# armlabstanford/Touch-GS

Hardware: AMD Instinct MI355X
Metric: train iters/s (whole-job views/s) + render Mpix/s, 1M Gaussians @ 1080p (higher is better)
Workload: dtype f32; 1 GPU; configs[2]: 1M Gaussians, 1080p, full Touch-GS train loop (RGB L1/SSIM + tactile depth/uncertainty loss), one view per rank per iter; gaussians=1000000, width=1920, height=1080, sh_degree=3, views=8, tiles=8160, longest_tile_list_any_view=792, max_list_hint=1022, parallelism=dp1, layout=morton (model.spatial_sort(): same scene, rows permuted), depth_loss_type=DEPTH_UNCERTAINTY_WEIGHTED_LOSS

## Files before the change

include/tgs.h:

```cpp
#ifndef TGS_H
#define TGS_H
#include <stddef.h>
#include <stdint.h>

#ifdef __cplusplus
extern "C" {
#endif

#define TGS_VERSION 320
#define TGS_BLOCK 16
#define TGS_SPLAT_FLOATS 12
#define TGS_PARTIAL_FLOATS 12
#define TGS_GROUP 256

typedef enum TgsStatus {
  TGS_OK = 0,
  TGS_E_ARG = -1,
  TGS_E_HIP = -2,
  TGS_E_CAPACITY = -3
} TgsStatus;

typedef struct TgsCamera {
  float viewmat[16];
  float fx, fy, cx, cy;
  int32_t W, H;
  float near_plane;
  float pix_center;
  float bg[3];
  float glob_scale;
  int32_t long_run;
} TgsCamera;

typedef struct TgsLossSpec {
  const float* gt_rgb;
  const float* gt_depth;
  const float* uncertainty;
  float l1_weight;
  float depth_weight;
  float uncertainty_weight;
  float eps;
} TgsLossSpec;

typedef struct TgsAdamSpec {
  float lr_means, lr_scales, lr_quats, lr_opac, lr_sh_dc, lr_sh_rest;
  float beta1, beta2, eps;
  float bias_corr1, bias_corr2;
  const float* device_bias_corr;
} TgsAdamSpec;

int tgs_version(void);
const char* tgs_last_error(void);

int tgs_calib_fma_stream(int n_iter, float* sink, int64_t* n_wave_instr , void* stream);

int tgs_num_groups(int N);
int tgs_num_tiles(int W, int H);
int tgs_num_bands(int W, int H);
int tgs_band_tiles(int W, int H, int band, int* tile0, int* tile1);
int tgs_tile_order_len(int W, int H);
int tgs_tile_counter_len(int W, int H);
int64_t tgs_tile_start_len(int W, int H);
size_t tgs_sort_scratch_bytes(int64_t capacity);

int tgs_project_fwd(const TgsCamera* cam , int N, const float* means,
                    const float* log_scales, const float* quats, const float* opac_logit,
                    const float* sh, int sh_stride, int sh_deg, const float* colors_in,
                    float* splats, int32_t* radii, void* stream);

int tgs_sh_fwd(int N, int sh_deg, int sh_stride, const float* dirs, const float* coeffs,
               float* colors, void* stream);
int tgs_sh_bwd(int N, int sh_deg, int sh_stride, const float* dirs, const float* v_colors,
               float* v_coeffs, void* stream);

int tgs_bin_sort(const TgsCamera* cam , int N, float* splats, int32_t* group_base,
                 int32_t* tile_start, int64_t tile_start_len, int32_t* tile_cursor, int32_t* sorted_gid,
                 int32_t* tile_order, int64_t capacity, void* scratch, int32_t* status,
                 int32_t* sticky_overflow, int32_t max_list_hint, void* stream);

int tgs_project_bin_sort(const TgsCamera* cam , int N, const float* means,
                         const float* log_scales, const float* quats, const float* opac_logit,
                         const float* sh, int sh_stride, int sh_deg, float* splats, int32_t* radii,
                         int32_t* group_base, int32_t* tile_start, int64_t tile_start_len, int32_t* tile_cursor,
                         int32_t* sorted_gid, int32_t* tile_order, int64_t capacity, void* scratch,
                         int32_t* status, int32_t* sticky_overflow, int32_t max_list_hint, void* stream);

int tgs_project_bin_sort_colors(const TgsCamera* cam , int N, const float* means,
                                const float* log_scales, const float* quats, const float* opac_logit,
                                const float* sh, int sh_stride, int sh_deg, float* splats,
                                int32_t* radii, int32_t* group_base, int32_t* tile_start, int64_t tile_start_len,
                                int32_t* tile_cursor, int32_t* sorted_gid, int32_t* tile_order,
                                int64_t capacity, void* scratch, int32_t* status,
                                int32_t* sticky_overflow, int32_t max_list_hint, const float* colors_in,
                                const int32_t* color_tag, int32_t tag_expect, void* stream);

typedef struct TgsRasterOpts {
  int32_t k6_blocks;
  int32_t k6_split;
  int32_t k7_front_to_back;
  int32_t k7_quad;
  int32_t k7_quad_min_walk;
  int32_t k7_blocks;
  int32_t k6_split_floor;
  int32_t k6_split_heads;
} TgsRasterOpts;

int tgs_rasterize_fwd(const TgsCamera* cam , const float* splats,
                      const int32_t* sorted_gid, int32_t* tile_start, int64_t tile_start_len,
                      const int32_t* tile_order, float* out_rgb, float* out_depth, float* final_T,
                      int32_t* final_idx , int32_t* stop_pos ,
                      uint64_t* slot_ok , const TgsRasterOpts* opts ,
                      void* stream);
size_t tgs_slot_ok_len(int W, int H, int64_t capacity);

int tgs_rasterize_depth_stats(const TgsCamera* cam , const float* splats, const int32_t* sorted_gid,
                              const int32_t* tile_start, int64_t tile_start_len, const int32_t* tile_order ,
                              const float* out_depth, const float* final_T, const int32_t* stop_pos ,
                              float* depth_var, float* median_depth, int32_t* median_gid ,
                              const TgsRasterOpts* opts , void* stream);

int tgs_set_raster_variant(int k6_blocks_on, int k7_front_to_back);

int tgs_set_k7_quad(int factor, int min_walk);

int tgs_set_k7_scan(int min_walk, int heads);

int tgs_set_long_run(int tiles);

int tgs_set_k6_split(int factor);
int tgs_set_k6_split_shape(int floor, int heads);

int tgs_rasterize_bwd(const TgsCamera* cam , const float* splats,
                      const int32_t* group_base, const int32_t* sorted_gid,
                      int32_t* tile_start, int64_t tile_start_len, const int32_t* tile_order ,
                      const float* out_rgb, const float* out_depth, const float* final_T,
                      const int32_t* stop_pos, const float* v_rgb, const float* v_depth, const float* v_alpha,
                      const TgsLossSpec* loss , float* partials, float* tile_loss,
                      const uint64_t* slot_ok , const TgsRasterOpts* opts ,
                      void* stream);

int tgs_rasterize_bwd_band(const TgsCamera* cam , const float* splats,
                      const int32_t* group_base, const int32_t* sorted_gid,
                      int32_t* tile_start, int64_t tile_start_len, const int32_t* tile_order ,
                      const float* out_rgb, const float* out_depth, const float* final_T,
                      const int32_t* stop_pos, const float* v_rgb, const float* v_depth, const float* v_alpha,
                      const TgsLossSpec* loss , float* partials, float* tile_loss,
                      int band, const uint64_t* slot_ok ,
                      const TgsRasterOpts* opts , void* stream);

int tgs_reduce_partials(int N, const float* splats, const int32_t* group_base,
                        const TgsCamera* cam , const float* partials, float* v_splats,
                        void* stream);

int tgs_project_bwd(const TgsCamera* cam , int N, const float* means,
                    const float* log_scales, const float* quats, const float* opac_logit,
                    const float* sh, int sh_stride, int sh_deg, const float* splats,
                    const int32_t* group_base, const float* partials, const float* v_splats,
                    float* v_means, float* v_log_scales, float* v_quats, float* v_opac_logit,
                    float* v_sh, float* v_xy,
                    const int32_t* skip_if_overflow , void* stream);

int tgs_project_bwd_adam(const TgsCamera* cam , int N, int sh_stride, int sh_deg,
                         float* params, float* exp_avg, float* exp_avg_sq,
                         const TgsAdamSpec* spec , const float* splats,
                         const int32_t* group_base, const float* partials, float* v_xy,
                         const int32_t* skip_if_overflow ,
                         void* stream);

int tgs_project_bwd_adam_next(const TgsCamera* cam , int N, int sh_stride, int sh_deg,
                              float* params, float* exp_avg, float* exp_avg_sq,
                              const TgsAdamSpec* spec , const float* splats,
                              const int32_t* group_base, const float* partials, float* v_xy,
                              const int32_t* skip_if_overflow ,
                              const TgsCamera* next_cam , float* colors_next,
                              int32_t* color_tag, int32_t tag_value, void* stream);

int tgs_project_bwd_adam_next_front(const TgsCamera* cam , int N, int sh_stride, int sh_deg,
                                    float* params, float* exp_avg, float* exp_avg_sq,
                                    const TgsAdamSpec* spec , const float* splats,
                                    const int32_t* group_base, const float* partials, float* v_xy,
                                    const int32_t* skip_if_overflow ,
                                    const TgsCamera* next_cam , float* colors_next,
                                    int32_t* tag_word, int32_t tag_value, float* splats_next,
                                    int32_t* radii_next, int32_t* group_base_next, int32_t* tile_cursor_next,
                                    int64_t capacity_next, void* scratch_next, int32_t* status_next,
                                    int32_t* sticky_overflow,
                                    int counters_cleared , void* stream);
int tgs_adam_geom_project_next(const TgsCamera* next_cam , int N, int sh_stride, int sh_deg,
                               float* params, const float* grads, float* exp_avg, float* exp_avg_sq,
                               const TgsAdamSpec* spec , float grad_scale,
                               const int32_t* skip_if_overflow, int32_t* tag_word, int32_t tag_value,
                               float* splats_next, int32_t* radii_next, int32_t* group_base_next,
                               int32_t* tile_cursor_next, int64_t capacity_next, void* scratch_next,
                               int32_t* status_next, int32_t* sticky_overflow, int counters_cleared, void* stream);
int tgs_adam_sh_gathered_geom_project_next(const TgsCamera* next_cam , int world, int N, int sh_stride, int sh_deg,
                                           float* params, const float* grads, int n_chunks,
                                           const int32_t* chunk_begin , const float* const* chunk_blocks ,
                                           float* exp_avg, float* exp_avg_sq, const TgsAdamSpec* spec ,
                                           float grad_scale, const int32_t* skip_if_overflow, int32_t* tag_word,
                                           int32_t tag_value, float* splats_next, int32_t* radii_next,
                                           int32_t* group_base_next, int32_t* tile_cursor_next, int64_t capacity_next,
                                           void* scratch_next, int32_t* status_next, int32_t* sticky_overflow,
                                           int counters_cleared, void* stream);
int tgs_project_bin_sort_front(const TgsCamera* cam , int N, const float* means,
                               const float* log_scales, const float* quats, const float* opac_logit,
                               const float* sh, int sh_stride, int sh_deg, float* splats, int32_t* radii,
                               int32_t* group_base, int32_t* tile_start, int64_t tile_start_len, int32_t* tile_cursor,
                               int32_t* sorted_gid, int32_t* tile_order, int64_t capacity, void* scratch,
                               int32_t* status, int32_t* sticky_overflow, int32_t max_list_hint,
                               const int32_t* tag_word, int32_t tag_expect,
                               const TgsCamera* next_cam , int32_t* next_tile_cursor ,
                               int32_t* next_status , void* stream);
int tgs_front_can_clear_next(int N, int W, int H);

int tgs_project_bwd_color(const TgsCamera* cam , int N, const float* means,
                          const float* log_scales, const float* quats, const float* opac_logit,
                          const float* sh, int sh_stride, int sh_deg, const float* splats,
                          const int32_t* group_base, const float* partials, float* v_means,
                          float* v_log_scales, float* v_quats, float* v_opac_logit, float* v_color,
                          float* v_xy, const int32_t* skip_if_overflow ,
                          void* stream);
int tgs_project_bwd_color_rows(const TgsCamera* cam , int N, int row_begin, int row_end,
                               const float* means, const float* log_scales, const float* quats,
                               const float* opac_logit, const float* sh, int sh_stride, int sh_deg,
                               const float* splats, const int32_t* group_base, const float* partials,
                               float* v_means, float* v_log_scales, float* v_quats, float* v_opac_logit,
                               float* v_color_rows, float* v_xy, const int32_t* skip_if_overflow, void* stream);
int tgs_adam_step_sh_gathered_rows(int world, int N, int row_begin, int row_end, int sh_stride, int sh_deg,
                                   float* params, const float* v_color_rows_all, float* exp_avg,
                                   float* exp_avg_sq, const TgsAdamSpec* spec , float grad_scale,
                                   const int32_t* skip_if_overflow, void* stream);
int tgs_dp_agree_overflow(int world, int N, const float* v_color_all, int32_t* status_out,
                          int32_t* sticky_overflow , void* stream);
int tgs_adam_step_sh_gathered(int world, int N, int sh_stride, int sh_deg, float* params,
                              const float* v_color_all, float* exp_avg, float* exp_avg_sq,
                              const TgsAdamSpec* spec , float grad_scale,
                              const int32_t* skip_if_overflow ,
                              void* stream);

int tgs_store_small(float* dst, const float* host_vals , int n, void* stream);

int tgs_adam_step(int N, int sh_stride, float* params, const float* grads, float* exp_avg,
                  float* exp_avg_sq, const TgsAdamSpec* spec , float grad_scale,
                  int64_t elem_begin, int64_t elem_end,
                  const int32_t* skip_if_overflow , void* stream);

int tgs_ssim_fwd_bwd(int W, int H, const float* img, const float* gt, float weight,
                     float* block_partials, float* v_img, float* scratch, void* stream);
int tgs_ssim_fwd_bwd_rows(int W, int H, const float* img, const float* gt, float weight,
                          float* block_partials, int n_partials, float* v_img, float* scratch,
                          int y0, int y1, int count_y0, int count_y1, void* stream);

int tgs_depth_corr_fwd_bwd(int W, int H, const float* out_depth, const float* final_T, const float* mono,
                           float alpha_min, float weight, float* tile_moments, float* stats,
                           float* v_depth , float* v_alpha , void* stream);

int tgs_depth_corr_local_fwd_bwd(int W, int H, const float* out_depth, const float* final_T, const float* mono,
                                 float alpha_min, float weight_global, float weight_local, int patch_tiles, int off_x,
                                 int off_y, int min_count, float min_var_ratio, float* tile_moments, float* patch_stats,
                                 float* stats , float* v_depth , float* v_alpha ,
                                 void* stream);

#define TGS_PEER_MEM_UNCACHED 1
#define TGS_PEER_MEM_FINEGRAINED 2
#define TGS_PEER_MEM_PLAIN 4
int tgs_peer_alloc(size_t bytes, int allow_kinds, void** dptr, unsigned char* handle64, int* kind_out );
int tgs_peer_open(const unsigned char* handle64, void** dptr);
int tgs_peer_close(void* dptr);
int tgs_peer_free(void* dptr);
int tgs_peer_push(int n_dst, void* const* dsts, int32_t* const* flags, const void* src, size_t bytes,
                  int32_t seq, int32_t* ticket, void* stream);
int tgs_peer_scatter(int n_dst, void* const* dsts, int32_t* const* flags, const void* src,
                     size_t slice_bytes, size_t total_bytes, int32_t seq, int32_t* ticket, void* stream);
int tgs_peer_reduce_push(int world, const void* const* srcs, int n_dst, void* const* dsts,
                         int32_t* const* flags, size_t bytes, int32_t seq, int32_t* ticket, void* stream);
int tgs_peer_signal(int n, int32_t* const* flags, int32_t seq, void* stream);
int tgs_peer_wait(int n, const int32_t* const* flags, int32_t seq, int32_t* err, float timeout_s,
                  int32_t* poison_a , int32_t* poison_b , void* stream);

#ifdef __cplusplus
}
#endif
#endif
```

touch_gs_amd/_lib.py:

```python
from __future__ import annotations

import ctypes as C
import os

_HERE = os.path.dirname(os.path.abspath(__file__))
LIB_PATH = os.environ.get("TGS_LIB_PATH") or os.path.join(_HERE, "lib", "libtgs_hip.so")

SPLAT_FLOATS = 12
PARTIAL_FLOATS = 12
GROUP = 256
BLOCK = 16


class TgsCamera(C.Structure):
    _fields_ = [("viewmat", C.c_float * 16), ("fx", C.c_float), ("fy", C.c_float),
                ("cx", C.c_float), ("cy", C.c_float), ("W", C.c_int32), ("H", C.c_int32),
                ("near_plane", C.c_float), ("pix_center", C.c_float), ("bg", C.c_float * 3),
                ("glob_scale", C.c_float), ("long_run", C.c_int32)]


class TgsLossSpec(C.Structure):
    _fields_ = [("gt_rgb", C.c_void_p), ("gt_depth", C.c_void_p), ("uncertainty", C.c_void_p),
                ("l1_weight", C.c_float), ("depth_weight", C.c_float),
                ("uncertainty_weight", C.c_float), ("eps", C.c_float)]


class TgsRasterOpts(C.Structure):
    _fields_ = [("k6_blocks", C.c_int32), ("k6_split", C.c_int32), ("k7_front_to_back", C.c_int32),
                ("k7_quad", C.c_int32), ("k7_quad_min_walk", C.c_int32), ("k7_blocks", C.c_int32),
                ("k6_split_floor", C.c_int32), ("k6_split_heads", C.c_int32)]


class TgsAdamSpec(C.Structure):
    _fields_ = [("lr_means", C.c_float), ("lr_scales", C.c_float), ("lr_quats", C.c_float),
                ("lr_opac", C.c_float), ("lr_sh_dc", C.c_float), ("lr_sh_rest", C.c_float),
                ("beta1", C.c_float), ("beta2", C.c_float), ("eps", C.c_float),
                ("bias_corr1", C.c_float), ("bias_corr2", C.c_float), ("device_bias_corr", C.c_void_p)]


_P = C.c_void_p
_I = C.c_int
SIGNATURES = {
    "tgs_version": (C.c_int, []),
    "tgs_last_error": (C.c_char_p, []),
    "tgs_calib_fma_stream": (C.c_int, [_I, _P, C.POINTER(C.c_int64), _P]),
    "tgs_num_groups": (C.c_int, [_I]),
    "tgs_num_tiles": (C.c_int, [_I, _I]),
    "tgs_tile_order_len": (C.c_int, [_I, _I]),
    "tgs_num_bands": (C.c_int, [_I, _I]),
    "tgs_band_tiles": (C.c_int, [_I, _I, _I, C.POINTER(C.c_int), C.POINTER(C.c_int)]),
    "tgs_tile_counter_len": (C.c_int, [_I, _I]),
    "tgs_tile_start_len": (C.c_int64, [_I, _I]),
    "tgs_sort_scratch_bytes": (C.c_size_t, [C.c_int64]),
    "tgs_project_fwd": (C.c_int, [C.POINTER(TgsCamera), _I, _P, _P, _P, _P, _P, _I, _I, _P, _P, _P, _P]),
    "tgs_sh_fwd": (C.c_int, [_I, _I, _I, _P, _P, _P, _P]),
    "tgs_sh_bwd": (C.c_int, [_I, _I, _I, _P, _P, _P, _P]),
    "tgs_bin_sort": (C.c_int, [C.POINTER(TgsCamera), _I, _P, _P, _P, C.c_int64, _P, _P, _P, C.c_int64, _P, _P, _P, C.c_int32, _P]),
    "tgs_project_bin_sort": (C.c_int, [C.POINTER(TgsCamera), _I, _P, _P, _P, _P, _P, _I, _I, _P, _P, _P, _P, C.c_int64, _P, _P,
                                       _P, C.c_int64, _P, _P, _P, C.c_int32, _P]),
    "tgs_project_bin_sort_colors": (C.c_int, [C.POINTER(TgsCamera), _I, _P, _P, _P, _P, _P, _I, _I, _P, _P, _P, _P, C.c_int64, _P,
                                              _P, _P, C.c_int64, _P, _P, _P, C.c_int32, _P, _P, C.c_int32, _P]),
    "tgs_rasterize_fwd": (C.c_int, [C.POINTER(TgsCamera), _P, _P, _P, C.c_int64, _P, _P, _P, _P, _P, _P, _P, C.POINTER(TgsRasterOpts), _P]),
    "tgs_rasterize_depth_stats": (C.c_int, [C.POINTER(TgsCamera), _P, _P, _P, C.c_int64] + [_P] * 7 + [C.POINTER(TgsRasterOpts), _P]),
    "tgs_set_raster_variant": (C.c_int, [_I, _I]),
    "tgs_set_k7_scan": (C.c_int, [_I, _I]),
    "tgs_set_k7_quad": (C.c_int, [_I, _I]),
    "tgs_set_k6_split": (C.c_int, [_I]),
    "tgs_set_long_run": (C.c_int, [_I]),
    "tgs_set_k6_split_shape": (C.c_int, [_I, _I]),
    "tgs_slot_ok_len": (C.c_size_t, [_I, _I, C.c_int64]),
    "tgs_rasterize_bwd": (C.c_int, [C.POINTER(TgsCamera)] + [_P] * 4 + [C.c_int64] + [_P] * 8 + [C.POINTER(TgsLossSpec), _P, _P, _P, C.POINTER(TgsRasterOpts), _P]),
    "tgs_rasterize_bwd_band": (C.c_int, [C.POINTER(TgsCamera)] + [_P] * 4 + [C.c_int64] + [_P] * 8 + [C.POINTER(TgsLossSpec), _P, _P, _I, _P, C.POINTER(TgsRasterOpts), _P]),
    "tgs_reduce_partials": (C.c_int, [_I, _P, _P, C.POINTER(TgsCamera), _P, _P, _P]),
    "tgs_project_bwd": (C.c_int, [C.POINTER(TgsCamera), _I, _P, _P, _P, _P, _P, _I, _I] + [_P] * 12),
    "tgs_project_bwd_adam": (C.c_int, [C.POINTER(TgsCamera), _I, _I, _I, _P, _P, _P, C.POINTER(TgsAdamSpec), _P, _P, _P, _P, _P, _P]),
    "tgs_project_bwd_adam_next": (C.c_int, [C.POINTER(TgsCamera), _I, _I, _I, _P, _P, _P, C.POINTER(TgsAdamSpec), _P, _P, _P,
                                            _P, _P, C.POINTER(TgsCamera), _P, _P, C.c_int32, _P]),
    "tgs_project_bwd_adam_next_front": (C.c_int, [C.POINTER(TgsCamera), _I, _I, _I, _P, _P, _P, C.POINTER(TgsAdamSpec), _P, _P, _P,
                                                  _P, _P, C.POINTER(TgsCamera), _P, _P, C.c_int32, _P, _P, _P, _P, C.c_int64,
                                                  _P, _P, _P, _I, _P]),
    "tgs_adam_geom_project_next": (C.c_int, [C.POINTER(TgsCamera), _I, _I, _I, _P, _P, _P, _P, C.POINTER(TgsAdamSpec), C.c_float,
                                             _P, _P, C.c_int32, _P, _P, _P, _P, C.c_int64, _P, _P, _P, _I, _P]),
    "tgs_adam_sh_gathered_geom_project_next": (C.c_int, [C.POINTER(TgsCamera), _I, _I, _I, _I, _P, _P, _I, C.POINTER(C.c_int32),
                                                         C.POINTER(C.c_void_p), _P, _P, C.POINTER(TgsAdamSpec), C.c_float, _P, _P,
                                                         C.c_int32, _P, _P, _P, _P, C.c_int64, _P, _P, _P, _I, _P]),
    "tgs_project_bin_sort_front": (C.c_int, [C.POINTER(TgsCamera), _I, _P, _P, _P, _P, _P, _I, _I, _P, _P, _P, _P, C.c_int64, _P,
                                             _P, _P, C.c_int64, _P, _P, _P, C.c_int32, _P, C.c_int32, C.POINTER(TgsCamera), _P, _P, _P]),
    "tgs_front_can_clear_next": (C.c_int, [_I, _I, _I]),
    "tgs_project_bwd_color": (C.c_int, [C.POINTER(TgsCamera), _I, _P, _P, _P, _P, _P, _I, _I] + [_P] * 11),
    "tgs_project_bwd_color_rows": (C.c_int, [C.POINTER(TgsCamera), _I, _I, _I, _P, _P, _P, _P, _P, _I, _I] + [_P] * 11),
    "tgs_adam_step_sh_gathered_rows": (C.c_int, [_I, _I, _I, _I, _I, _I, _P, _P, _P, _P, C.POINTER(TgsAdamSpec), C.c_float, _P, _P]),
    "tgs_dp_agree_overflow": (C.c_int, [_I, _I, _P, _P, _P, _P]),
    "tgs_adam_step_sh_gathered": (C.c_int, [_I, _I, _I, _I, _P, _P, _P, _P, C.POINTER(TgsAdamSpec), C.c_float, _P, _P]),
    "tgs_store_small": (C.c_int, [_P, C.POINTER(C.c_float), _I, _P]),
    "tgs_adam_step": (C.c_int, [_I, _I, _P, _P, _P, _P, C.POINTER(TgsAdamSpec), C.c_float, C.c_int64, C.c_int64, _P, _P]),
    "tgs_ssim_fwd_bwd": (C.c_int, [_I, _I, _P, _P, C.c_float, _P, _P, _P, _P]),
    "tgs_ssim_fwd_bwd_rows": (C.c_int, [_I, _I, _P, _P, C.c_float, _P, _I, _P, _P, _I, _I, _I, _I, _P]),
    "tgs_depth_corr_fwd_bwd": (C.c_int, [_I, _I, _P, _P, _P, C.c_float, C.c_float, _P, _P, _P, _P, _P]),
    "tgs_depth_corr_local_fwd_bwd": (C.c_int, [_I, _I, _P, _P, _P, C.c_float, C.c_float, C.c_float, _I, _I, _I, _I, C.c_float,
                                              _P, _P, _P, _P, _P, _P]),
    "tgs_peer_alloc": (C.c_int, [C.c_size_t, _I, C.POINTER(C.c_void_p), C.POINTER(C.c_ubyte), C.POINTER(C.c_int)]),
    "tgs_peer_open": (C.c_int, [C.POINTER(C.c_ubyte), C.POINTER(C.c_void_p)]),
    "tgs_peer_close": (C.c_int, [_P]),
    "tgs_peer_free": (C.c_int, [_P]),
    "tgs_peer_push": (C.c_int, [_I, C.POINTER(C.c_void_p), C.POINTER(C.c_void_p), _P, C.c_size_t, C.c_int32, _P, _P]),
    "tgs_peer_scatter": (C.c_int, [_I, C.POINTER(C.c_void_p), C.POINTER(C.c_void_p), _P, C.c_size_t, C.c_size_t, C.c_int32, _P, _P]),
    "tgs_peer_reduce_push": (C.c_int, [_I, C.POINTER(C.c_void_p), _I, C.POINTER(C.c_void_p), C.POINTER(C.c_void_p), C.c_size_t,
                                       C.c_int32, _P, _P]),
    "tgs_peer_signal": (C.c_int, [_I, C.POINTER(C.c_void_p), C.c_int32, _P]),
    "tgs_peer_wait": (C.c_int, [_I, C.POINTER(C.c_void_p), C.c_int32, _P, C.c_float, _P, _P, _P]),
}

_lib = None


def load():
    global _lib
    if _lib is not None:
        return _lib
    if not os.path.exists(LIB_PATH):
        raise ImportError(
            f"{LIB_PATH} not found: build it with `python -c 'import __graft_entry__ as g; g.build()'` "
            "or touch_gs_amd/csrc/build.sh (hipcc --offload-arch=gfx950). touch_gs_amd has no CPU fallback.")
    lib = C.CDLL(LIB_PATH)
    for name, (res, args) in SIGNATURES.items():
        fn = getattr(lib, name)
        fn.restype = res
        fn.argtypes = args
    _lib = lib
    return lib


def check(rc: int, what: str = ""):
    if rc != 0:
        msg = load().tgs_last_error().decode(errors="replace")
        raise RuntimeError(f"libtgs_hip {what} failed ({rc}): {msg}")


def ptr(t):
    if t is None:
        return None
    if not t.is_cuda:
        raise RuntimeError("touch_gs_amd ops need device (HIP) tensors; there is no CPU path")
    if not t.is_contiguous():
        raise RuntimeError("touch_gs_amd ops need contiguous tensors")
    if t.numel() == 0:
        return _dummy(t.device).data_ptr()
    return t.data_ptr()


_DUMMY = {}


def _dummy(device):
    import torch
    key = str(device)
    if key not in _DUMMY:
        _DUMMY[key] = torch.zeros(64, dtype=torch.float32, device=device)
    return _DUMMY[key]
```

touch_gs_amd/csrc/imgloss.hip:

```cpp
#include <math.h>
#include <stdlib.h>
#include "tgs_common.h"

namespace {

constexpr int WIN = 11, HALO = 5;
struct Win { float g[WIN]; };
#ifdef TGS_SSIM_SGPR_WINDOW
#define WK(k) win.g[k]
#else
__device__ constexpr float WGT[WIN] = {0x1.0d956cp-10f, 0x1.f1fe02p-8f, 0x1.26eb18p-5f, 0x1.bff0fep-4f, 0x1.b43c4p-3f,
                                       0x1.10656p-2f, 0x1.b43c4p-3f, 0x1.bff0fep-4f, 0x1.26eb18p-5f, 0x1.f1fe02p-8f,
                                       0x1.0d956cp-10f};
#define WK(k) WGT[k]
#endif

#ifndef TGS_SSIM_DMA
#define TGS_SSIM_DMA 0
#endif
constexpr int SW = 64;
constexpr int NTH = 3 * SW;
constexpr int RB = WIN;
__host__ __device__ constexpr int seg_rows(int nblk) { return RB * nblk - 2 * HALO; }

template <int CH>
struct RowBlock {
  static constexpr int ROWF = (SW + 2 * HALO) * CH;
  static constexpr int NIT = (RB * ROWF + NTH - 1) / NTH;
  template <int B = 8>
  static __device__ __forceinline__ void stage(const float* __restrict__ src, float* __restrict__ lds,
                                               int W, int H, int x0, int r0, int tid) {
#pragma unroll 1
    for (int it0 = 0; it0 < NIT; it0 += B) {
      float v[B];
#pragma unroll
      for (int u = 0; u < B; u++) {
        const int i = tid + NTH * (it0 + u);
        const int j = i / ROWF, e = i - j * ROWF;
        const int gy = r0 + j, gxf = (x0 - HALO) * CH + e;
        v[u] = 0.f;
        if (i < RB * ROWF && gy >= 0 && gy < H && gxf >= 0 && gxf < W * CH) v[u] = src[(size_t)gy * W * CH + gxf];
      }
#pragma unroll
      for (int u = 0; u < B; u++) {
        const int i = tid + NTH * (it0 + u);
        if (i < RB * ROWF) lds[i] = v[u];
      }
    }
  }
  static constexpr int PADF = (RB * ROWF + TGS_WAVE - 1) / TGS_WAVE * TGS_WAVE;
  static constexpr int NDMA = PADF / TGS_WAVE;
  static __device__ __forceinline__ void dma(__amdgpu_buffer_rsrc_t rsrc, float* __restrict__ lds, int W, int H, int x0, int r0, int tid) {
    typedef __attribute__((address_space(3))) float lds_float;
    const int wave = __builtin_amdgcn_readfirstlane(tid >> 6), lane = tid & 63;
    constexpr int NW = NTH / TGS_WAVE;
    const int gx0 = (x0 - HALO) * CH, WC = W * CH;
#pragma unroll
    for (int u = 0; u * NW < NDMA; u++) {
      const int chunk = u * NW + wave;
      if (chunk < NDMA) {
        const int i = chunk * TGS_WAVE + lane;
        const int j = i / ROWF, e = i - j * ROWF;
        const int gy = r0 + j, gxf = gx0 + e;
        const bool in = i < RB * ROWF && (unsigned)gy < (unsigned)H && (unsigned)gxf < (unsigned)WC;
        const unsigned off = in ? (unsigned)(gy * WC + gxf) * 4u : 0xffffffffu;
        __builtin_amdgcn_raw_ptr_buffer_load_lds(rsrc, (lds_float*)(lds + chunk * TGS_WAVE), 4, off, 0, 0, 0);
      }
    }
  }
  static __device__ __forceinline__ void stage2(const float* __restrict__ src_a, const float* __restrict__ src_b,
                                                float* __restrict__ lds_a, float* __restrict__ lds_b,
                                                int W, int H, int x0, int r0, int tid) {
#ifndef TGS_SSIM_FWD_B
#define TGS_SSIM_FWD_B 13
#endif
    constexpr int B = TGS_SSIM_FWD_B;
#pragma unroll 1
    for (int it0 = 0; it0 < NIT; it0 += B) {
      float va[B], vb[B];
#pragma unroll
      for (int u = 0; u < B; u++) {
        const int i = tid + NTH * (it0 + u);
        const int j = i / ROWF, e = i - j * ROWF;
        const int gy = r0 + j, gxf = (x0 - HALO) * CH + e;
        va[u] = 0.f; vb[u] = 0.f;
        if (it0 + u < NIT && i < RB * ROWF && gy >= 0 && gy < H && gxf >= 0 && gxf < W * CH) {
          const size_t o = (size_t)gy * W * CH + gxf;
          va[u] = src_a[o]; vb[u] = src_b[o];
        }
      }
#pragma unroll
      for (int u = 0; u < B; u++) {
        const int i = tid + NTH * (it0 + u);
        if (it0 + u < NIT && i < RB * ROWF) { lds_a[i] = va[u]; lds_b[i] = vb[u]; }
      }
    }
  }
};

__global__ __launch_bounds__(NTH) __attribute__((amdgpu_waves_per_eu(4, 8))) void k_ssim_fwd(int W, int H, Win win,
                                                  const float* __restrict__ img,
                                                  const float* __restrict__ gt,
                                                  float* __restrict__ adj ,
                                                  float* __restrict__ block_partials, int n_partials, int NBLK,
                                                  int y_lo, int y_hi, int c_lo, int c_hi) {
  const int SEG = seg_rows(NBLK);
  constexpr int ROWF = RowBlock<3>::ROWF;
#if TGS_SSIM_DMA & 1
  __shared__ float sa2[2][RowBlock<3>::PADF], sb2[2][RowBlock<3>::PADF];
  const __amdgpu_buffer_rsrc_t rs_a = __builtin_amdgcn_make_buffer_rsrc((void*)img, 0, (int)((size_t)W * H * 12), 0x00020000);
  const __amdgpu_buffer_rsrc_t rs_b = __builtin_amdgcn_make_buffer_rsrc((void*)gt, 0, (int)((size_t)W * H * 12), 0x00020000);
#else
  __shared__ float sa[RB * ROWF], sb[RB * ROWF];
#endif
  __shared__ float red[NTH / TGS_WAVE];
  const int tid = threadIdx.x;
  const int x0 = blockIdx.x * SW, ys = y_lo + blockIdx.y * SEG;
  const int gx = x0 + tid / 3, c = tid - (tid / 3) * 3;
  const int ye = min(ys + SEG, y_hi);
  float w[RB][5];
#pragma unroll
  for (int p = 0; p < RB; p++)
#pragma unroll
    for (int q = 0; q < 5; q++) w[p][q] = 0.f;
  float msum = 0.f;
#if TGS_SSIM_DMA & 1
  RowBlock<3>::dma(rs_a, sa2[0], W, H, x0, ys - HALO, tid);
  RowBlock<3>::dma(rs_b, sb2[0], W, H, x0, ys - HALO, tid);
#endif
  for (int blk = 0; blk < NBLK; blk++) {
    const int r0 = ys - HALO + blk * RB;
    if (r0 - HALO >= ye) break;
#if TGS_SSIM_DMA & 1
    asm volatile("s_waitcnt vmcnt(0)" ::: "memory");
    __syncthreads();
    if (blk + 1 < NBLK && r0 + RB - HALO < ye) {
      RowBlock<3>::dma(rs_a, sa2[(blk + 1) & 1], W, H, x0, r0 + RB, tid);
      RowBlock<3>::dma(rs_b, sb2[(blk + 1) & 1], W, H, x0, r0 + RB, tid);
    }
    const float* sa = sa2[blk & 1];
    const float* sb = sb2[blk & 1];
#else
    __syncthreads();
    {
      RowBlock<3>::stage2(img, gt, sa, sb, W, H, x0, r0, tid);
    }
    __syncthreads();
#endif
#pragma unroll
    for (int p = 0; p < RB; p++) {
      const float* ra = sa + p * ROWF + tid;
      const float* rb = sb + p * ROWF + tid;
      float m1 = 0.f, m2 = 0.f, e11 = 0.f, e22 = 0.f, e12 = 0.f;
#pragma unroll
      for (int k = 0; k < WIN; k++) {
        const float a = ra[3 * k], b = rb[3 * k];
        const float ga = WK(k) * a, gb = WK(k) * b;
        m1 += ga; m2 += gb;
        e11 = fmaf(ga, a, e11); e22 = fmaf(gb, b, e22); e12 = fmaf(ga, b, e12);
      }
      w[p][0] = m1; w[p][1] = m2; w[p][2] = e11; w[p][3] = e22; w[p][4] = e12;
      const int gy = r0 + p - HALO;
      if (gy >= ys && gy < ye) {
        float o[5] = {0.f, 0.f, 0.f, 0.f, 0.f};
#pragma unroll
        for (int k = 0; k < WIN; k++) {
#pragma unroll
          for (int q = 0; q < 5; q++) o[q] = fmaf(WK(k), w[(p + 1 + k) % RB][q], o[q]);
        }
        const float C1 = 0.01f * 0.01f, C2 = 0.03f * 0.03f;
        const float mu1 = o[0], mu2 = o[1];
        const float s11 = o[2] - mu1 * mu1, s22 = o[3] - mu2 * mu2, s12 = o[4] - mu1 * mu2;
        const float n1 = 2.f * mu1 * mu2 + C1, n2 = 2.f * s12 + C2;
        const float d1 = mu1 * mu1 + mu2 * mu2 + C1, d2 = s11 + s22 + C2;
        const float id1 = __builtin_amdgcn_rcpf(d1), id2 = __builtin_amdgcn_rcpf(d2);
        const float m = n1 * n2 * id1 * id2;
        if (gx < W) {
          if (gy >= c_lo && gy < c_hi) msum += m;
          if (adj) {
            const float dm_ds12 = 2.f * n1 * id1 * id2;
            const float dm_ds11 = -m * id2;
            const float dm_dmu1 = 2.f * mu2 * n2 * id1 * id2 - m * 2.f * mu1 * id1;
            float* o3 = adj + (((size_t)gy * W + gx) * 3 + c) * 3;
            o3[0] = dm_dmu1 - 2.f * mu1 * dm_ds11 - mu2 * dm_ds12;
            o3[1] = dm_ds11;
            o3[2] = dm_ds12;
          }
        }
      }
    }
  }
  const float tot = wave_sum(msum);
  if ((tid & 63) == 0) red[tid >> 6] = tot;
  __syncthreads();
  const int wg = blockIdx.y * gridDim.x + blockIdx.x, nwg = gridDim.x * gridDim.y;
  if (tid == 0) block_partials[wg] = red[0] + red[1] + red[2];
  for (int i = nwg + wg * NTH + tid; i < n_partials; i += nwg * NTH) block_partials[i] = 0.f;
}

__global__ __launch_bounds__(NTH) __attribute__((amdgpu_waves_per_eu(4, 8))) void k_ssim_bwd(int W, int H, Win win, float weight,
                                                  const float* __restrict__ img,
                                                  const float* __restrict__ gt,
                                                  const float* __restrict__ adj,
                                                  float* __restrict__ v_img, int NBLK, int y_lo, int y_hi) {
  const int SEG = seg_rows(NBLK);
  constexpr int ROWF = RowBlock<9>::ROWF;
#if TGS_SSIM_DMA & 2
  __shared__ float sadj2[2][RowBlock<9>::PADF];
  const __amdgpu_buffer_rsrc_t rs_j = __builtin_amdgcn_make_buffer_rsrc((void*)adj, 0, (int)((size_t)W * H * 36), 0x00020000);
#else
  __shared__ float sadj[RB * ROWF];
#endif
  const int tid = threadIdx.x;
  const int x0 = blockIdx.x * SW, ys = y_lo + blockIdx.y * SEG;
  const int gx = x0 + tid / 3;
  const int ye = min(ys + SEG, y_hi);
  float w[RB][3];
#pragma unroll
  for (int p = 0; p < RB; p++) { w[p][0] = 0.f; w[p][1] = 0.f; w[p][2] = 0.f; }
#if TGS_SSIM_DMA & 2
  RowBlock<9>::dma(rs_j, sadj2[0], W, H, x0, ys - HALO, tid);
#endif
  for (int blk = 0; blk < NBLK; blk++) {
    const int r0 = ys - HALO + blk * RB;
    if (r0 - HALO >= ye) break;
#if TGS_SSIM_DMA & 2
    asm volatile("s_waitcnt vmcnt(0)" ::: "memory");
    __syncthreads();
    if (blk + 1 < NBLK && r0 + RB - HALO < ye) RowBlock<9>::dma(rs_j, sadj2[(blk + 1) & 1], W, H, x0, r0 + RB, tid);
    const float* sadj = sadj2[blk & 1];
#else
    __syncthreads();
    {
#ifndef TGS_SSIM_BWD_B
#define TGS_SSIM_BWD_B 20
#endif
      RowBlock<9>::stage<TGS_SSIM_BWD_B>(adj, sadj, W, H, x0, r0, tid);
    }
    __syncthreads();
#endif
#pragma unroll
    for (int p = 0; p < RB; p++) {
      const float* r = sadj + p * ROWF + 3 * tid;
      float h0 = 0.f, h1 = 0.f, h2 = 0.f;
#pragma unroll
      for (int k = 0; k < WIN; k++) {
        h0 = fmaf(WK(k), r[9 * k], h0);
        h1 = fmaf(WK(k), r[9 * k + 1], h1);
        h2 = fmaf(WK(k), r[9 * k + 2], h2);
      }
      w[p][0] = h0; w[p][1] = h1; w[p][2] = h2;
      const int gy = r0 + p - HALO;
      if (gy >= ys && gy < ye) {
        float o0 = 0.f, o1 = 0.f, o2 = 0.f;
#pragma unroll
        for (int k = 0; k < WIN; k++) {
          o0 = fmaf(WK(k), w[(p + 1 + k) % RB][0], o0);
          o1 = fmaf(WK(k), w[(p + 1 + k) % RB][1], o1);
          o2 = fmaf(WK(k), w[(p + 1 + k) % RB][2], o2);
        }
        if (gx < W) {
          const size_t pidx = (size_t)gy * W * 3 + (size_t)x0 * 3 + tid;
          v_img[pidx] = weight * (o0 + 2.f * img[pidx] * o1 + gt[pidx] * o2);
        }
      }
    }
  }
}


constexpr int SWO = SW - 2 * HALO;
__host__ __device__ constexpr int fused_seg_rows(int nblk) { return RB * nblk - 4 * HALO; }

__global__ __launch_bounds__(NTH) __attribute__((amdgpu_waves_per_eu(3, 4))) void k_ssim_fused(
    int W, int H, float weight, const float* __restrict__ img, const float* __restrict__ gt,
    float* __restrict__ v_img, float* __restrict__ block_partials, int n_partials, int NBLK,
    int y_lo, int y_hi, int c_lo, int c_hi) {
  const int SEG = fused_seg_rows(NBLK);
  constexpr int ROWF = RowBlock<3>::ROWF;
  constexpr int ADJF = SW * 9;
  __shared__ float sa[RB * ROWF], sb[RB * ROWF];
  __shared__ float sadj[RB * ADJF];
  __shared__ float red[NTH / TGS_WAVE];
  const int tid = threadIdx.x;
  const int col = tid / 3, c = tid - col * 3;
  const int xa0 = blockIdx.x * SWO - HALO;
  const int gx = xa0 + col;
  const int ys = y_lo + blockIdx.y * SEG, ye = min(ys + SEG, y_hi);
  const bool own_col = col >= HALO && col < SW - HALO;
  const int cb = min(max(col - HALO, 0), SWO - 1);
  float w[RB][5], w2[RB][3];
#pragma unroll
  for (int p = 0; p < RB; p++) {
#pragma unroll
    for (int q = 0; q < 5; q++) w[p][q] = 0.f;
    w2[p][0] = 0.f; w2[p][1] = 0.f; w2[p][2] = 0.f;
  }
  float msum = 0.f;
  for (int blk = 0; blk < NBLK; blk++) {
    const int r0 = ys - 2 * HALO + blk * RB;
    if (r0 - 2 * HALO >= ye) break;
    __syncthreads();
    RowBlock<3>::stage2(img, gt, sa, sb, W, H, xa0, r0, tid);
    __syncthreads();
#pragma unroll
    for (int p = 0; p < RB; p++) {
      const float* ra = sa + p * ROWF + tid;
      const float* rb = sb + p * ROWF + tid;
      float m1 = 0.f, m2 = 0.f, e11 = 0.f, e22 = 0.f, e12 = 0.f;
#pragma unroll
      for (int k = 0; k < WIN; k++) {
        const float a = ra[3 * k], b = rb[3 * k];
        const float ga = WK(k) * a, gb = WK(k) * b;
        m1 += ga; m2 += gb;
        e11 = fmaf(ga, a, e11); e22 = fmaf(gb, b, e22); e12 = fmaf(ga, b, e12);
      }
      w[p][0] = m1; w[p][1] = m2; w[p][2] = e11; w[p][3] = e22; w[p][4] = e12;
      const int gy = r0 + p - HALO;
      float A = 0.f, B = 0.f, C = 0.f;
      if (gy >= ys - HALO && gy < ye + HALO && gy >= 0 && gy < H) {
        float o[5] = {0.f, 0.f, 0.f, 0.f, 0.f};
#pragma unroll
        for (int k = 0; k < WIN; k++) {
#pragma unroll
          for (int q = 0; q < 5; q++) o[q] = fmaf(WK(k), w[(p + 1 + k) % RB][q], o[q]);
        }
        const float C1 = 0.01f * 0.01f, C2 = 0.03f * 0.03f;
        const float mu1 = o[0], mu2 = o[1];
        const float s11 = o[2] - mu1 * mu1, s22 = o[3] - mu2 * mu2, s12 = o[4] - mu1 * mu2;
        const float n1 = 2.f * mu1 * mu2 + C1, n2 = 2.f * s12 + C2;
        const float d1 = mu1 * mu1 + mu2 * mu2 + C1, d2 = s11 + s22 + C2;
        const float id1 = __builtin_amdgcn_rcpf(d1), id2 = __builtin_amdgcn_rcpf(d2);
        const float m = n1 * n2 * id1 * id2;
        if (gx >= 0 && gx < W) {
          if (own_col && gy >= ys && gy < ye && gy >= c_lo && gy < c_hi) msum += m;
          const float dm_ds12 = 2.f * n1 * id1 * id2;
          const float dm_ds11 = -m * id2;
          const float dm_dmu1 = 2.f * mu2 * n2 * id1 * id2 - m * 2.f * mu1 * id1;
          A = dm_dmu1 - 2.f * mu1 * dm_ds11 - mu2 * dm_ds12;
          B = dm_ds11;
          C = dm_ds12;
        }
      }
      float* o3 = sadj + p * ADJF + tid * 3;
      o3[0] = A; o3[1] = B; o3[2] = C;
    }
    __syncthreads();
#pragma unroll
    for (int p = 0; p < RB; p++) {
      const float* r = sadj + p * ADJF + (cb * 3 + c) * 3;
      float h0 = 0.f, h1 = 0.f, h2 = 0.f;
#pragma unroll
      for (int k = 0; k < WIN; k++) {
        h0 = fmaf(WK(k), r[9 * k], h0);
        h1 = fmaf(WK(k), r[9 * k + 1], h1);
        h2 = fmaf(WK(k), r[9 * k + 2], h2);
      }
      w2[p][0] = h0; w2[p][1] = h1; w2[p][2] = h2;
      const int gy = r0 + p - 2 * HALO;
      if (gy >= ys && gy < ye) {
        float o0 = 0.f, o1 = 0.f, o2 = 0.f;
#pragma unroll
        for (int k = 0; k < WIN; k++) {
          o0 = fmaf(WK(k), w2[(p + 1 + k) % RB][0], o0);
          o1 = fmaf(WK(k), w2[(p + 1 + k) % RB][1], o1);
          o2 = fmaf(WK(k), w2[(p + 1 + k) % RB][2], o2);
        }
        if (own_col && gx < W) {
          const size_t pidx = ((size_t)gy * W + gx) * 3 + c;
          v_img[pidx] = weight * (o0 + 2.f * img[pidx] * o1 + gt[pidx] * o2);
        }
      }
    }
  }
  const float tot = wave_sum(msum);
  if ((tid & 63) == 0) red[tid >> 6] = tot;
  __syncthreads();
  const int wg = blockIdx.y * gridDim.x + blockIdx.x, nwg = gridDim.x * gridDim.y;
  if (tid == 0) block_partials[wg] = red[0] + red[1] + red[2];
  for (int i = nwg + wg * NTH + tid; i < n_partials; i += nwg * NTH) block_partials[i] = 0.f;
}

}

static inline bool count_inside(int y0, int y1, int c0, int c1) { return c0 >= c1 || (c0 >= y0 && c1 <= y1); }

static int ssim_impl(int W, int H, const float* img, const float* gt, float weight,
                     float* block_partials, int n_partials, float* v_img, float* scratch,
                     int y0, int y1, int c0, int c1, void* stream) {
  TGS_CHECK_ARG(W > 0 && H > 0, "bad image size");
  TGS_CHECK_ARG(img && gt && block_partials, "null pointer");
  TGS_CHECK_ARG(!v_img || scratch, "gradient needs scratch");
  TGS_CHECK_ARG(0 <= y0 && y0 <= y1 && y1 <= H && y0 <= c0 && c0 <= c1 && c1 <= y1, "bad row range");
  Win win;
  double g[WIN], sum = 0.0;
  for (int i = 0; i < WIN; i++) { g[i] = exp(-(double)((i - HALO) * (i - HALO)) / (2.0 * 1.5 * 1.5)); sum += g[i]; }
  for (int i = 0; i < WIN; i++) win.g[i] = (float)(g[i] / sum);
  static const int env_nblk = [] { const char* e = getenv("TGS_SSIM_NBLK"); return e ? max(2, min(16, atoi(e))) : 0; }();
  static const int env_fused = [] { const char* e = getenv("TGS_SSIM_FUSED"); return e ? atoi(e) : 0; }();
  if (v_img && env_fused && y1 > y0 && count_inside(y0, y1, c0, c1)) {
    const int fx = (W + SWO - 1) / SWO;
    auto wgs = [&](int nb) { return (long long)fx * ((y1 - y0 + fused_seg_rows(nb) - 1) / fused_seg_rows(nb)); };
    int nblk = 7;
    while (nblk > 3 && wgs(nblk) < 600) nblk--;
    if (env_nblk) nblk = max(3, env_nblk);
    while (nblk < 16 && wgs(nblk) > n_partials) nblk++;
    TGS_CHECK_ARG(wgs(nblk) <= n_partials, "block_partials too small");
    const int SEGF = fused_seg_rows(nblk);
    hipLaunchKernelGGL(k_ssim_fused, dim3(fx, (y1 - y0 + SEGF - 1) / SEGF, 1), dim3(NTH), 0, (hipStream_t)stream, W, H, weight,
                       img, gt, v_img, block_partials, n_partials, nblk, y0, y1, c0, c1);
    TGS_CHECK_LAUNCH();
    return TGS_OK;
  }
  const int f0 = v_img ? max(0, y0 - HALO) : y0, f1 = v_img ? min(H, y1 + HALO) : y1;
  const int rows = f1 - f0;
  if (rows <= 0) return TGS_OK;
  const int sx = (W + SW - 1) / SW;
  int nblk = 4;
  while (nblk > 2 && (long long)sx * ((rows + seg_rows(nblk) - 1) / seg_rows(nblk)) < 3 * 256) nblk--;
  if (env_nblk) nblk = env_nblk;
  while (nblk < 16 && (long long)sx * ((rows + seg_rows(nblk) - 1) / seg_rows(nblk)) > n_partials) nblk++;
  TGS_CHECK_ARG((long long)sx * ((rows + seg_rows(nblk) - 1) / seg_rows(nblk)) <= n_partials, "block_partials too small");
  const int SEG = seg_rows(nblk);
  const dim3 block(NTH);
  hipStream_t s = (hipStream_t)stream;
  hipLaunchKernelGGL(k_ssim_fwd, dim3(sx, (rows + SEG - 1) / SEG, 1), block, 0, s, W, H, win, img, gt,
                     v_img ? scratch : nullptr, block_partials, n_partials, nblk, f0, f1, c0, c1);
  TGS_CHECK_LAUNCH();
  if (v_img && y1 > y0) {
    hipLaunchKernelGGL(k_ssim_bwd, dim3(sx, (y1 - y0 + SEG - 1) / SEG, 1), block, 0, s, W, H, win, weight, img, gt,
                       scratch, v_img, nblk, y0, y1);
    TGS_CHECK_LAUNCH();
  }
  return TGS_OK;
}

extern "C" int tgs_ssim_fwd_bwd(int W, int H, const float* img, const float* gt, float weight,
                                float* block_partials, float* v_img, float* scratch,
                                void* stream) {
  return ssim_impl(W, H, img, gt, weight, block_partials, ((W + 15) / 16) * ((H + 15) / 16), v_img, scratch,
                   0, H, 0, H, stream);
}

extern "C" int tgs_ssim_fwd_bwd_rows(int W, int H, const float* img, const float* gt, float weight,
                                     float* block_partials, int n_partials, float* v_img,
                                     float* scratch, int y0, int y1, int count_y0, int count_y1,
                                     void* stream) {
  return ssim_impl(W, H, img, gt, weight, block_partials, n_partials, v_img, scratch, y0, y1, count_y0,
                   count_y1, stream);
}
```

touch_gs_amd/csrc/raster.hip:

```cpp
#include <stdlib.h>
#include <type_traits>
#include "tgs_common.h"

namespace {

constexpr float ALPHA_MAX = 0.999f;
constexpr float CLAMP_FREE_OPACITY = 0.99f;
constexpr float T_STOP = 1e-4f;
constexpr float LOG2E = 1.4426950408889634f;
constexpr float LOG2_255 = 7.994353436858858f;

__device__ __forceinline__ int xcd_tile(int b, int T) {
  return tgs_xcd_slot_tile(T, b & 7, b >> 3);
}

typedef unsigned tgs_u2v __attribute__((ext_vector_type(2)));
__device__ __forceinline__ float fold_xor16(float v) {
  const tgs_u2v r = __builtin_amdgcn_permlane16_swap(__float_as_uint(v), __float_as_uint(v), false, false);
  return __uint_as_float(r.x) + __uint_as_float(r.y);
}
__device__ __forceinline__ float fold_xor32(float v) {
  const tgs_u2v r = __builtin_amdgcn_permlane32_swap(__float_as_uint(v), __float_as_uint(v), false, false);
  return __uint_as_float(r.x) + __uint_as_float(r.y);
}

struct LossK {
  const float* gt_rgb;
  const float* gt_depth;
  const float* unc;
  float l1w, dw, uw, eps;
  int on;
};

struct TileRec {
  float4 a;
  float4 b;
  float4 c;
};

__device__ __forceinline__ void centre_rel(float4 r0, float4 r2, int tx, int ty, float pix_center, float& gx, float& gy) {
  const unsigned rect = __float_as_uint(r2.z);
  const int dx = tx - (int)(rect & 255u), dy = ty - (int)((rect >> 8) & 255u);
  gx = r0.x - ((float)(dx * TGS_BLOCK) + (7.5f + pix_center));
  gy = r0.y - ((float)(dy * TGS_BLOCK) + (7.5f + pix_center));
}

template <bool QUAD_MASK = true>
__device__ __forceinline__ TileRec make_tile_rec(float4 r0, float4 r1, float4 r2, float gx, float gy) {
  const float A = r1.x, B = r1.y, Cc = r1.z;
  const float L = -__log2f(r0.w);
  TileRec t;
  t.a.x = LOG2E * (0.5f * A * gx * gx + B * gx * gy + 0.5f * Cc * gy * gy) + L;
  t.a.y = -LOG2E * (A * gx + B * gy);
  t.a.z = -LOG2E * (B * gx + Cc * gy);
  t.a.w = 0.5f * LOG2E * A;
  t.b.x = LOG2E * B;
  t.b.y = 0.5f * LOG2E * Cc;
  t.b.z = r0.z;
  t.b.w = r1.w;
  unsigned mask = 0u;
  const float slack = LOG2_255 + 1e-3f;
  if (QUAD_MASK && L < LOG2_255) {
    const float c0 = t.a.x, c1 = t.a.y, c2 = t.a.z, c3 = t.a.w, c4 = t.b.x, c5 = t.b.y;
    const float ic3 = __builtin_amdgcn_rcpf(c3), ic5 = __builtin_amdgcn_rcpf(c5);
#pragma unroll
    for (int k = 0; k < 4; k++) {
      const float u0 = (k & 1) ? 0.5f : -7.5f, u1 = u0 + 7.f;
      const float v0 = (k >> 1) ? 0.5f : -7.5f, v1 = v0 + 7.f;
      float best;
      if (gx >= u0 && gx <= u1 && gy >= v0 && gy <= v1) {
        best = L;
      } else {
        best = 3.0e38f;
#pragma unroll
        for (int e = 0; e < 2; e++) {
          const float v = e ? v1 : v0;
          const float lin = fmaf(c4, v, c1);
          const float us = fminf(fmaxf(-0.5f * lin * ic3, u0), u1);
          best = fminf(best, fmaf(us, fmaf(c3, us, lin), fmaf(v, fmaf(c5, v, c2), c0)));
          const float u = e ? u1 : u0;
          const float lin2 = fmaf(c4, u, c2);
          const float vs = fminf(fmaxf(-0.5f * lin2 * ic5, v0), v1);
          best = fminf(best, fmaf(vs, fmaf(c5, vs, lin2), fmaf(u, fmaf(c3, u, c1), c0)));
        }
      }
      mask |= (best <= slack) ? (1u << k) : 0u;
    }
  }
  t.c = make_float4(r2.x, r2.y, 0.f, __uint_as_float(mask));
  return t;
}

struct PixConst {
  float u[2], v[2], uu[2], vv[2], uv[4];
};

__device__ __forceinline__ PixConst make_pix_const(int lane) {
  PixConst p;
  p.u[0] = (float)(lane & 7) - 7.5f; p.u[1] = p.u[0] + 8.f;
  p.v[0] = (float)(lane >> 3) - 7.5f; p.v[1] = p.v[0] + 8.f;
#pragma unroll
  for (int i = 0; i < 2; i++) { p.uu[i] = p.u[i] * p.u[i]; p.vv[i] = p.v[i] * p.v[i]; }
#pragma unroll
  for (int k = 0; k < 4; k++) p.uv[k] = p.u[k & 1] * p.v[k >> 1];
  return p;
}

__device__ __forceinline__ float eval_s(const float4& a, const float4& b, const PixConst& p, int k) {
  float s = fmaf(a.y, p.u[k & 1], a.x);
  s = fmaf(a.z, p.v[k >> 1], s);
  s = fmaf(a.w, p.uu[k & 1], s);
  s = fmaf(b.x, p.uv[k], s);
  s = fmaf(b.y, p.vv[k >> 1], s);
  return s;
}

__device__ __forceinline__ size_t slot_ok_index(int batch_pos, int tile) {
  return (size_t)(batch_pos >> 6) + (size_t)tile;
}

#define TGS_NO_STOP 0x7fffffff
__device__ __forceinline__ float stop_code(int pos) { return __uint_as_float(0xC0000000u | (unsigned)pos); }
__device__ __forceinline__ int stop_of(float smax) {
  return smax > 0.f ? TGS_NO_STOP : (int)(__float_as_uint(smax) & 0x3fffffffu);
}
__device__ __forceinline__ float batch_stop_code(int j) { return __uint_as_float(0xE0000000u | (unsigned)j); }
__device__ __forceinline__ float finish_batch_stop(float smax, int batch_rel) {
  const unsigned b = __float_as_uint(smax);
  return (b & 0xffffff00u) == 0xE0000000u ? stop_code(batch_rel + (int)(b & 0xffu)) : smax;
}

__device__ __forceinline__ int32_t* frame_scratch(const int32_t* tile_start) { return const_cast<int32_t*>(tile_start); }
__device__ __forceinline__ void publish_walk(const int32_t* __restrict__ tile_start, int T_total, const float (&smax)[4],
                                             int n, int lane) {
  int wl = 0;
#pragma unroll
  for (int k = 0; k < 4; k++)
    wl = max(wl, smax[k] == -3.0e38f ? 0 : min(stop_of(smax[k]), n));
  wl = wave_minmax_i<true>(wl);
  if (lane == 0 && wl > 0) {
    const int xcc = (int)(__builtin_amdgcn_s_getreg(20 | (0 << 6) | ((4 - 1) << 11)) & (TGS_WALK_WORDS - 1));
    atomicMax(frame_scratch(tile_start) + TGS_WALK_AT(T_total, xcc), wl);
    atomicAdd(frame_scratch(tile_start) + TGS_WALKSUM_AT(T_total, xcc), wl);
  }
}

template <bool MAYCLAMP = true, int WANT_OK = 0>
__device__ __forceinline__ float blend_step(float s, float& T, float& smax, float& Tnew, bool& go,
                                            unsigned long long& okb, float stopv = -3.0e38f) {
  const float e = __builtin_amdgcn_exp2f(-s);
  const float al = MAYCLAMP ? fminf(ALPHA_MAX, e) : e;
  const bool ok = s <= smax;
  if constexpr (WANT_OK == 1) okb = __builtin_amdgcn_ballot_w64(ok);
  Tnew = fmaf(-al, T, T);
  const bool above = Tnew > T_STOP;
// ... 668 lines not shown
      w = (red_c == 7) ? v0 : w;
      w = (red_c == 6 || red_c == 8) ? 8.f : w;
      w = (red_c == 9) ? u0 * u0 : w;
      w = (red_c == 11) ? v0 * v0 : w;
      w = (red_c == 10) ? 16.f * u0 + 64.f : w;
      w = (red_c == 12) ? 16.f * v0 + 64.f : w;
      w = (red_c >= 14) ? 0.f : w;
      wt[i] = w;
    }
  }
  const float4 z4 = make_float4(0.f, 0.f, 0.f, 0.f);
  int base = start;
  for (; base < end; base += 64) {
    unsigned slot_live = 0u;
#pragma unroll
    for (int k = 0; k < 4; k++) slot_live |= (__ballot(smax[k] > 0.f) != 0ull) ? (1u << k) : 0u;
    if (slot_live == 0u) break;
    const int cnt = min(64, end - base);
    size_t P = 0;
    float4 a0 = z4, a1 = z4;
    unsigned my_mask = 0u;
    __syncthreads();
    if (lane < cnt) {
      const int gid = sorted_gid[base + lane];
      const float* r = splats + (size_t)gid * TGS_SPLAT_FLOATS;
      a0 = ld4(r); a1 = ld4(r + 4);
      const float4 a2 = ld4(r + 8);
      float gx, gy;
      centre_rel(a0, a2, tx, ty, cam.pix_center, gx, gy);
      a0.x = gx; a0.y = gy;
      const TileRec t = make_tile_rec(a0, a1, a2, gx, gy);
      recs[lane * 3] = t.a; recs[lane * 3 + 1] = t.b; recs[lane * 3 + 2] = t.c;
      my_mask = __float_as_uint(t.c.w);
      P = pair_index(group_base, gid, a2, tx, ty);
    }
    sums[lane * 4] = z4; sums[lane * 4 + 1] = z4; sums[lane * 4 + 2] = z4; sums[lane * 4 + 3] = z4;
    __syncthreads();

    unsigned long long qm[4];
#pragma unroll
    for (int k = 0; k < 4; k++)
      qm[k] = ((slot_live >> k) & 1u) ? __ballot((my_mask >> k) & 1u) : 0ull;
    if (slot_ok) {
      const unsigned long long* o = slot_ok + 4 * slot_ok_index(base, tile);
#pragma unroll
      for (int k = 0; k < 4; k++) qm[k] &= __builtin_nontemporal_load(o + k);
    }
    auto walk = [&](auto mayclamp) {
    constexpr bool MAYCLAMP = decltype(mayclamp)::value;
    unsigned long long rem = qm[0] | qm[1] | qm[2] | qm[3];
    while (rem) {
      const int j = __builtin_ctzll(rem);
      rem &= rem - 1;
      const unsigned m = (unsigned)((qm[0] >> j) & 1ull) | ((unsigned)((qm[1] >> j) & 1ull) << 1) |
                         ((unsigned)((qm[2] >> j) & 1ull) << 2) | ((unsigned)((qm[3] >> j) & 1ull) << 3);
      const float4 qa = recs[j * 3], qb = recs[j * 3 + 1], qc = recs[j * 3 + 2];
      float acc[RED_ROWS];
#pragma unroll
      for (int c = 0; c < RED_ROWS; c++) acc[c] = 0.f;
      unsigned long long any = 0ull;
#pragma unroll
      for (int k = 0; k < 4; k++) {
        if (m & (1u << k)) {
          const float s = eval_s(qa, qb, pc, k);
          float Tn; bool go;
          unsigned long long okb;
          const float al = blend_step<MAYCLAMP, 2>(s, T[k], smax[k], Tn, go, okb);
          const float w = al * T[k];
          const float kap = w * __builtin_amdgcn_rcpf(Tn);
          acc[0] = fmaf(w, vCr[k], acc[0]); acc[1] = fmaf(w, vCg[k], acc[1]);
          acc[2] = fmaf(w, vCb[k], acc[2]); acc[3] = fmaf(w, vD[k], acc[3]);
          float cv = qb.w * vCr[k];
          cv = fmaf(qc.x, vCg[k], cv); cv = fmaf(qc.y, vCb[k], cv); cv = fmaf(qb.z, vD[k], cv);
          const float z = w * cv;
          XP[k] += z;
          float q = fmaf(kap, XP[k], z);
          if constexpr (MAYCLAMP) q *= fmaxf(__builtin_amdgcn_exp2f(-s) * (1.0f / ALPHA_MAX), 1.0f);
          T[k] = fmaf(-al, T[k], T[k]);
          acc[4] += q;
          if (k & 1) acc[5] += q;
          if (k >> 1) acc[6] += q;
          acc[7] = fmaf(q, pc.uv[k], acc[7]);
          any |= okb;
        }
      }
      if (any != 0ull) {
#pragma unroll
        for (int c = 0; c < RED_ROWS; c++) red[c * RED_RS + lane] = acc[c];
        __builtin_amdgcn_fence(__ATOMIC_RELEASE, "wavefront");
        __builtin_amdgcn_wave_barrier();
        __builtin_amdgcn_fence(__ATOMIC_ACQUIRE, "wavefront");
        const float4 r0 = ld4(red_rd), r1 = ld4(red_rd + 4), r2 = ld4(red_rd + 8), r3 = ld4(red_rd + 12);
        float o0 = r0.x * wt[0], o1 = r1.x * wt[4], o2 = r2.x * wt[8], o3 = r3.x * wt[12];
        o0 = fmaf(r0.y, wt[1], o0); o1 = fmaf(r1.y, wt[5], o1); o2 = fmaf(r2.y, wt[9], o2); o3 = fmaf(r3.y, wt[13], o3);
        o0 = fmaf(r0.z, wt[2], o0); o1 = fmaf(r1.z, wt[6], o1); o2 = fmaf(r2.z, wt[10], o2); o3 = fmaf(r3.z, wt[14], o3);
        o0 = fmaf(r0.w, wt[3], o0); o1 = fmaf(r1.w, wt[7], o1); o2 = fmaf(r2.w, wt[11], o2); o3 = fmaf(r3.w, wt[15], o3);
        float O = (o0 + o1) + (o2 + o3);
        O = fold_xor16(O);
        O = fold_xor32(O);
        if (lane < 16) reinterpret_cast<float*>(sums)[j * 16 + lane] = O;
        __builtin_amdgcn_wave_barrier();
      }
    }
    };
    if (__ballot(lane < cnt && a0.w > CLAMP_FREE_OPACITY) != 0ull) walk(std::true_type{});
    else walk(std::false_type{});
    __syncthreads();
    if (lane < cnt) {
      const float4 s0 = sums[lane * 4], s1 = sums[lane * 4 + 1], s2 = sums[lane * 4 + 2], s3 = sums[lane * 4 + 3];
      const float gx = a0.x, gy = a0.y;
      const float A = a1.x, B = a1.y, Cc = a1.z;
      const float Q0 = s1.x, Qu = s1.y + s1.z, Qv = s1.w + s2.x, Quu = s2.y + s2.z, Qvv = s2.w + s3.x, Quv = s3.y;
      const float Mx = -(gx * Q0 - Qu), My = -(gy * Q0 - Qv);
      const float Mxx = -(gx * gx * Q0 - 2.f * gx * Qu + Quu);
      const float Mxy = -(gx * gy * Q0 - gx * Qv - gy * Qu + Quv);
      const float Myy = -(gy * gy * Q0 - 2.f * gy * Qv + Qvv);
      float* o = partials + P * TGS_PARTIAL_FLOATS;
      st4(o, make_float4(A * Mx + B * My, B * Mx + Cc * My, s0.w, Q0 / a0.w));
      st4(o + 4, make_float4(0.5f * Mxx, Mxy, 0.5f * Myy, s0.x));
      st4(o + 8, make_float4(s0.y, s0.z, 0.f, 0.f));
    }
  }
  for (int i = base + lane; i < end; i += 64) {
    const int gid = sorted_gid[i];
    const size_t P = pair_index(group_base, gid, ld4(splats + (size_t)gid * TGS_SPLAT_FLOATS + 8), tx, ty);
    float* o = partials + P * TGS_PARTIAL_FLOATS;
    st4(o, z4); st4(o + 4, z4); st4(o + 8, z4);
  }
}


struct QuadRule { int factor, min_walk, scan_min, scan_heads; };
__device__ __forceinline__ bool frame_is_chain_bound(const int32_t* __restrict__ tile_start, int T, QuadRule q) {
  if (q.factor <= 0) return false;
  int walk = 0;
  long long work = 0;
#pragma unroll
  for (int i = 0; i < TGS_WALK_WORDS; i++) {
    walk = max(walk, tile_start[TGS_WALK_AT(T, i)]);
    work += tile_start[TGS_WALKSUM_AT(T, i)];
  }
  return (long long)walk * 8192 > work * q.factor;
}

#ifndef TGS_K7_FIRSTQ
#define TGS_K7_FIRSTQ 0
#endif
#ifndef TGS_K7_RECPF
#define TGS_K7_RECPF 0
#endif
#ifndef TGS_K7_PAIR
#define TGS_K7_PAIR 0
#endif
#if TGS_K7_RECPF
__attribute__((amdgpu_waves_per_eu(4, 8)))
#endif
__global__ __launch_bounds__(64) void k_raster_bwd(
    CamK cam, int T_total, const float* __restrict__ splats, const int32_t* __restrict__ group_base,
    const int32_t* __restrict__ sorted_gid, const int32_t* __restrict__ tile_start,
    const float* __restrict__ out_rgb, const float* __restrict__ out_depth,
    const float* __restrict__ final_T, const int32_t* __restrict__ stop_pos, const float* __restrict__ v_rgb,
    const float* __restrict__ v_depth, const float* __restrict__ v_alpha, LossK loss,
    float* __restrict__ partials, float* __restrict__ tile_loss,
    const int32_t* __restrict__ tile_order, QuadRule quad) {
  if (blockIdx.x == 0 && threadIdx.x < TGS_WALK_WORDS && quad.factor > 0)
    frame_scratch(tile_start)[TGS_SLOTCTR_AT(T_total, threadIdx.x)] = 0;
  const int tile = tile_order ? tile_order[blockIdx.x] : xcd_tile(blockIdx.x, T_total);
  if (tile >= T_total) return;
  const int lane = threadIdx.x;
  const int ty = tile / cam.TW, tx = tile - ty * cam.TW;
  const PixConst pc = make_pix_const(lane);
  const int start = tile_start[tile], end = tile_start[tile + 1];
  const int n = end - start;

  float T[4] = {1.f, 1.f, 1.f, 1.f};
  float vCr[4], vCg[4], vCb[4], vD[4], SX[4];
  int lim[4];
  float l_l1 = 0.f, l_dep = 0.f;
#pragma unroll
  for (int k = 0; k < 4; k++) {
    const int px = tx * TGS_BLOCK + 8 * (k & 1) + (lane & 7);
    const int py = ty * TGS_BLOCK + 8 * (k >> 1) + (lane >> 3);
    lim[k] = 0; vCr[k] = vCg[k] = vCb[k] = vD[k] = SX[k] = 0.f;
    if (px < cam.W && py < cam.H) {
      const size_t p = (size_t)py * cam.W + px;
      const float Tf = final_T[p];
      T[k] = Tf;
      lim[k] = min(stop_pos[p], n);
      float vA = v_alpha ? v_alpha[p] : 0.f;
      if (v_rgb) { vCr[k] = v_rgb[3 * p]; vCg[k] = v_rgb[3 * p + 1]; vCb[k] = v_rgb[3 * p + 2]; }
      if (v_depth) vD[k] = v_depth[p];
      if (loss.on) {
        if (loss.gt_rgb) {
          const float d0 = out_rgb[3 * p] - loss.gt_rgb[3 * p];
          const float d1 = out_rgb[3 * p + 1] - loss.gt_rgb[3 * p + 1];
          const float d2 = out_rgb[3 * p + 2] - loss.gt_rgb[3 * p + 2];
          vCr[k] += loss.l1w * ((d0 > 0.f) - (d0 < 0.f));
          vCg[k] += loss.l1w * ((d1 > 0.f) - (d1 < 0.f));
          vCb[k] += loss.l1w * ((d2 > 0.f) - (d2 < 0.f));
          l_l1 += loss.l1w * (fabsf(d0) + fabsf(d1) + fabsf(d2));
        }
        if (loss.gt_depth) {
          const float gd = loss.gt_depth[p];
          if (gd > 0.f) {
            const float alpha = fmaxf(1.f - Tf, 1e-10f);
            const float ia = 1.0f / alpha;
            const float dhat = out_depth[p] * ia;
            const float r = dhat - gd;
            float wgt = loss.dw;
            if (loss.unc) wgt = wgt / (loss.uw * loss.unc[p] + loss.eps);
            l_dep += wgt * r * r;
            const float gdh = 2.f * wgt * r;
            vD[k] += gdh * ia;
            if (1.f - Tf > 1e-10f) vA += -gdh * dhat * ia;
          }
        }
      }
      const float bgdot = cam.bg[0] * vCr[k] + cam.bg[1] * vCg[k] + cam.bg[2] * vCb[k];
      SX[k] = -Tf * (vA - bgdot);
    }
  }
  if (tile_loss) {
    const float a = wave_sum(l_l1), b = wave_sum(l_dep);
    if (lane == 0) { tile_loss[2 * tile] = a; tile_loss[2 * tile + 1] = b; }
  }
  if (n == 0) return;
  int qlim[4];
#pragma unroll
  for (int k = 0; k < 4; k++) qlim[k] = wave_minmax_i<true>(lim[k]);
  const int tmax = max(max(qlim[0], qlim[1]), max(qlim[2], qlim[3]));
  if (tmax > quad.min_walk && frame_is_chain_bound(tile_start, T_total, quad)) return;
  const float4 z4 = make_float4(0.f, 0.f, 0.f, 0.f);
  for (int i = start + tmax + lane; i < end; i += 64) {
    const int gid = sorted_gid[i];
    const size_t P = pair_index(group_base, gid, ld4(splats + (size_t)gid * TGS_SPLAT_FLOATS + 8), tx, ty);
    float* o = partials + P * TGS_PARTIAL_FLOATS;
    st4(o, z4); st4(o + 4, z4); st4(o + 8, z4);
  }
  if (tmax == 0) return;

  __shared__ float4 recs[64 * 3];
  __shared__ float4 sums[64 * 4];
  constexpr int RED_RS = 68;
  constexpr int RED_ROWS = 8;
  __shared__ float4 red4[(TGS_K7_PAIR ? 2 : 1) * RED_ROWS * RED_RS / 4];
  float* red = reinterpret_cast<float*>(red4);
  const int red_c = lane & 15;
  const int red_part = (lane >> 4) ^ ((red_c >= 4 && red_c < 12) ? 1 : 0);
  float wt[16];
  const float* red_rd;
  {
    const unsigned long long ROWS = 0x0076454645443210ull;
    red_rd = red + (int)((ROWS >> (4 * red_c)) & 15ull) * RED_RS + red_part * 16;
#pragma unroll
    for (int i = 0; i < 16; i++) {
      const float u0 = (float)(i & 7) - 7.5f;
      const float v0 = (float)(2 * red_part + (i >> 3)) - 7.5f;
      float w = 1.f;
      w = (red_c == 5) ? u0 : w;
      w = (red_c == 7) ? v0 : w;
      w = (red_c == 6 || red_c == 8) ? 8.f : w;
      w = (red_c == 9) ? u0 * u0 : w;
      w = (red_c == 11) ? v0 * v0 : w;
      w = (red_c == 10) ? 16.f * u0 + 64.f : w;
      w = (red_c == 12) ? 16.f * v0 + 64.f : w;
      w = (red_c >= 14) ? 0.f : w;
      wt[i] = w;
    }
  }
  for (int base = start + ((tmax - 1) & ~63); base >= start; base -= 64) {
    const int rel = base - start;
    const int cnt = min(64, tmax - rel);
    size_t P = 0;
    float4 a0 = z4, a1 = z4;
    unsigned my_mask = 0u;
    __syncthreads();
    if (lane < cnt) {
      const int gid = sorted_gid[base + lane];
      const float* r = splats + (size_t)gid * TGS_SPLAT_FLOATS;
      a0 = ld4(r); a1 = ld4(r + 4);
      const float4 a2 = ld4(r + 8);
      float gx, gy;
      centre_rel(a0, a2, tx, ty, cam.pix_center, gx, gy);
      a0.x = gx; a0.y = gy;
      const TileRec t = make_tile_rec(a0, a1, a2, gx, gy);
      my_mask = __float_as_uint(t.c.w);
      recs[lane * 3] = t.a; recs[lane * 3 + 1] = t.b; recs[lane * 3 + 2] = t.c;
      P = pair_index(group_base, gid, a2, tx, ty);
    }
    sums[lane * 4] = z4; sums[lane * 4 + 1] = z4; sums[lane * 4 + 2] = z4; sums[lane * 4 + 3] = z4;
    __syncthreads();

    unsigned long long qm[4];
#pragma unroll
    for (int k = 0; k < 4; k++) {
      const int r = qlim[k] - rel;
      const unsigned long long keep = r >= 64 ? ~0ull : (r <= 0 ? 0ull : ((1ull << r) - 1ull));
      qm[k] = __ballot((my_mask >> k) & 1u) & keep;
    }
    const unsigned long long rem0 = qm[0] | qm[1] | qm[2] | qm[3];
    auto walk = [&](auto mayclamp) {
    constexpr bool MAYCLAMP = decltype(mayclamp)::value;
    unsigned long long rem = rem0;
    auto blend = [&](int j, const float4 qa, const float4 qb, const float4 qc, float (&acc)[RED_ROWS], unsigned long long& any) {
      const unsigned m = (unsigned)((qm[0] >> j) & 1ull) | ((unsigned)((qm[1] >> j) & 1ull) << 1) |
                         ((unsigned)((qm[2] >> j) & 1ull) << 2) | ((unsigned)((qm[3] >> j) & 1ull) << 3);
      const int pos = rel + j;
      any = 0ull;
      auto quad = [&](auto KC, auto FC) {
        constexpr int k = decltype(KC)::value;
        constexpr bool FIRST = decltype(FC)::value;
        const float s = eval_s(qa, qb, pc, k);
        const float e = __builtin_amdgcn_exp2f(-s);
        const float al0 = MAYCLAMP ? fminf(ALPHA_MAX, e) : e;
        const bool ok = s <= LOG2_255, in = pos < lim[k];
        const bool go = ok & in;
        const unsigned long long gob = __builtin_amdgcn_ballot_w64(ok) & __builtin_amdgcn_ballot_w64(in);
        const float al = go ? al0 : 0.f;
        const float ra = __builtin_amdgcn_rcpf(1.0f - al);
        const float Tp = T[k] * ra;
        const float w = al * Tp;
        float cv = qb.w * vCr[k];
        cv = fmaf(qc.x, vCg[k], cv); cv = fmaf(qc.y, vCb[k], cv); cv = fmaf(qb.z, vD[k], cv);
        const float z = w * cv;
        float q = fmaf(-(al * ra), SX[k], z);
        if constexpr (MAYCLAMP) q *= fmaxf(e * (1.0f / ALPHA_MAX), 1.0f);
        SX[k] += z;
        T[k] = Tp;
        if constexpr (FIRST) {
          acc[0] = w * vCr[k]; acc[1] = w * vCg[k]; acc[2] = w * vCb[k]; acc[3] = w * vD[k];
          acc[4] = q;
          acc[5] = (k & 1) ? q : 0.f;
          acc[6] = (k >> 1) ? q : 0.f;
          acc[7] = q * pc.uv[k];
        } else {
          acc[0] = fmaf(w, vCr[k], acc[0]); acc[1] = fmaf(w, vCg[k], acc[1]);
          acc[2] = fmaf(w, vCb[k], acc[2]); acc[3] = fmaf(w, vD[k], acc[3]);
          acc[4] += q;
          if (k & 1) acc[5] += q;
          if (k >> 1) acc[6] += q;
          acc[7] = fmaf(q, pc.uv[k], acc[7]);
        }
        any |= gob;
      };
#if TGS_K7_FIRSTQ
      using I0 = std::integral_constant<int, 0>; using I1 = std::integral_constant<int, 1>;
      using I2 = std::integral_constant<int, 2>; using I3 = std::integral_constant<int, 3>;
      const std::true_type F{}; const std::false_type A{};
      switch (__builtin_ctz(m | 16u)) {
        case 0: quad(I0{}, F); if (m & 2u) quad(I1{}, A); if (m & 4u) quad(I2{}, A); if (m & 8u) quad(I3{}, A); break;
        case 1: quad(I1{}, F); if (m & 4u) quad(I2{}, A); if (m & 8u) quad(I3{}, A); break;
        case 2: quad(I2{}, F); if (m & 8u) quad(I3{}, A); break;
        case 3: quad(I3{}, F); break;
        default:
#pragma unroll
          for (int c = 0; c < RED_ROWS; c++) acc[c] = 0.f;
      }
#else
#pragma unroll
      for (int c = 0; c < RED_ROWS; c++) acc[c] = 0.f;
      if (m & 1u) quad(std::integral_constant<int, 0>{}, std::false_type{});
      if (m & 2u) quad(std::integral_constant<int, 1>{}, std::false_type{});
      if (m & 4u) quad(std::integral_constant<int, 2>{}, std::false_type{});
      if (m & 8u) quad(std::integral_constant<int, 3>{}, std::false_type{});
#endif
    };
    auto reduce_rows = [&](const float* rd) {
      const float4 r0 = ld4(rd), r1 = ld4(rd + 4), r2 = ld4(rd + 8), r3 = ld4(rd + 12);
      float o0 = r0.x * wt[0], o1 = r1.x * wt[4], o2 = r2.x * wt[8], o3 = r3.x * wt[12];
      o0 = fmaf(r0.y, wt[1], o0); o1 = fmaf(r1.y, wt[5], o1); o2 = fmaf(r2.y, wt[9], o2); o3 = fmaf(r3.y, wt[13], o3);
      o0 = fmaf(r0.z, wt[2], o0); o1 = fmaf(r1.z, wt[6], o1); o2 = fmaf(r2.z, wt[10], o2); o3 = fmaf(r3.z, wt[14], o3);
      o0 = fmaf(r0.w, wt[3], o0); o1 = fmaf(r1.w, wt[7], o1); o2 = fmaf(r2.w, wt[11], o2); o3 = fmaf(r3.w, wt[15], o3);
      return (o0 + o1) + (o2 + o3);
    };
#if TGS_K7_RECPF
    if (rem == 0ull) return;
    int jn = 63 - __builtin_clzll(rem);
    rem &= ~(1ull << jn);
    float4 na = recs[jn * 3], nb = recs[jn * 3 + 1], nc = recs[jn * 3 + 2];
    for (;;) {
      const int j = jn;
      const float4 qa = na, qb = nb, qc = nc;
      const bool more = rem != 0ull;
      if (more) {
        jn = 63 - __builtin_clzll(rem);
        rem &= ~(1ull << jn);
        na = recs[jn * 3]; nb = recs[jn * 3 + 1]; nc = recs[jn * 3 + 2];
      }
      float acc[RED_ROWS];
      unsigned long long any;
      blend(j, qa, qb, qc, acc, any);
      if (any != 0ull) {
#pragma unroll
        for (int c = 0; c < RED_ROWS; c++) red[c * RED_RS + lane] = acc[c];
        __builtin_amdgcn_fence(__ATOMIC_RELEASE, "wavefront");
        __builtin_amdgcn_wave_barrier();
        __builtin_amdgcn_fence(__ATOMIC_ACQUIRE, "wavefront");
        float O = reduce_rows(red_rd);
// ... 833 lines not shown
          float* o = slab + src * SCAN_ENT;
          const int v0 = ((row & 1) << 1) | (row >> 1);
          o[v0] = f0; o[4 + v0] = f1; o[8 + (row >> 1)] = f2;
        }
      }
    };
    if (clampy) chunks(std::true_type{}); else chunks(std::false_type{});
    __syncthreads();
    {
      const float* o = acc + (bi & 1) * SCAN_ACC + li * SCAN_SLAB + (4 * w + row) * SCAN_ENT;
      const float4 x0 = ld4(o), x1 = ld4(o + 4);
      const float2 x2 = *reinterpret_cast<const float2*>(o + 8);
      float c[10] = {x0.x, x0.y, x0.z, x0.w, x1.x, x1.y, x1.z, x1.w, x2.x, x2.y};
      row_sum16x10(c);
      if (head) {
        float* t = tot + ((bi & 1) * 64 + 4 * w + row) * SCAN_ENT;
        st4(t, make_float4(c[0], c[1], c[2], c[3])); st4(t + 4, make_float4(c[4], c[5], c[6], c[7]));
        *reinterpret_cast<float2*>(t + 8) = make_float2(c[8], c[9]);
      }
    }
    if (bi > 0 && w == ((bi - 1) & 15)) finish(bi - 1);
    pP = P; pA = a1.x; pB = a1.y; pC = a1.z; pgx = gx; pgy = gy; popac = a0.w; pvalid = valid;
  }
  __syncthreads();
  if (w == ((nb - 1) & 15)) finish(nb - 1);
}

}

static TgsDefault g_k6_blocks{"TGS_K6_BLOCKS", 1, true};
static TgsDefault g_k7_f2b{"TGS_K7_F2B", 0, true};
static TgsDefault g_k7_quad{"TGS_K7_QUAD", 8, false, 255};
static TgsDefault g_k7_quad_min{"TGS_K7_QUAD_MIN", 16, false, (1 << 23) - 1};
static TgsDefault g_k6_split{"TGS_K6_SPLIT", 2, false};
static TgsDefault g_k7_blocks{"TGS_K7_BLOCKS", 0, true};
static TgsDefault g_k7_scan_min{"TGS_K7_SCAN_MIN", 0, false, 65535};
static TgsDefault g_k7_scan_heads{"TGS_K7_SCAN_HEADS", 512, false, 32767};
static TgsDefault g_k7_scan_side{"TGS_K7_SCAN_SIDE", 1, true};
struct ScanSide { hipStream_t s = nullptr; hipEvent_t fork = nullptr, join = nullptr; bool ok = false; };
static ScanSide& scan_side() {
  static ScanSide x = [] {
    ScanSide y;
    int lo = 0, hi = 0;
    y.ok = hipDeviceGetStreamPriorityRange(&lo, &hi) == hipSuccess &&
           hipStreamCreateWithPriority(&y.s, hipStreamNonBlocking, hi) == hipSuccess &&
           hipEventCreateWithFlags(&y.fork, hipEventDisableTiming) == hipSuccess &&
           hipEventCreateWithFlags(&y.join, hipEventDisableTiming) == hipSuccess;
    return y;
  }();
  return x;
}
static inline int opt_or(const TgsRasterOpts* o, int32_t TgsRasterOpts::*f, TgsDefault& d) {
  return (o && o->*f >= 0) ? (int)(o->*f) : d.get();
}
extern "C" int tgs_set_raster_variant(int k6_blocks_on, int k7_front_to_back) {
  if (k6_blocks_on >= 0) g_k6_blocks.set(k6_blocks_on);
  if (k7_front_to_back >= 0) g_k7_f2b.set(k7_front_to_back);
  return (g_k6_blocks.get() ? 1 : 0) | (g_k7_f2b.get() ? 2 : 0);
}
static TgsDefault g_k6_floor{"TGS_K6_FLOOR", 256, false, 65535};
static TgsDefault g_k6_heads{"TGS_K6_HEADS", 512, false, 32767};
extern "C" int tgs_set_k6_split_shape(int floor, int heads) {
  if (floor >= 0) g_k6_floor.set(floor);
  if (heads >= 0) g_k6_heads.set(heads);
  return g_k6_floor.get() | (g_k6_heads.get() << 16);
}
extern "C" int tgs_set_k6_split(int factor) {
  if (factor >= 0) g_k6_split.set(factor);
  return g_k6_split.get();
}
extern "C" int tgs_set_k7_scan(int min_walk, int heads) {
  if (min_walk >= 0) g_k7_scan_min.set(min_walk);
  if (heads >= 0) g_k7_scan_heads.set(heads);
  return g_k7_scan_min.get() | (g_k7_scan_heads.get() << 16);
}
#ifdef TGS_QUAD_TIMING
extern "C" int tgs_debug_quad_timing(unsigned long long* host_dst, int clear) {
  if (host_dst && hipMemcpyFromSymbol(host_dst, HIP_SYMBOL(g_quad_dbg), sizeof(unsigned long long) * 8192 * 16) != hipSuccess) return -1;
  if (clear) { void* p = nullptr; if (hipGetSymbolAddress(&p, HIP_SYMBOL(g_quad_dbg)) != hipSuccess || hipMemset(p, 0, sizeof(unsigned long long) * 8192 * 16) != hipSuccess) return -2; }
  return 0;
}
#endif
extern "C" int tgs_set_k7_quad(int factor, int min_walk) {
  if (factor >= 0) g_k7_quad.set(factor);
  if (min_walk >= 0) g_k7_quad_min.set(min_walk);
  return g_k7_quad.get() | (g_k7_quad_min.get() << 8);
}

extern "C" int tgs_rasterize_fwd(const TgsCamera* cam, const float* splats,
                                 const int32_t* sorted_gid, int32_t* tile_start, int64_t tile_start_len,
                                 const int32_t* tile_order, float* out_rgb, float* out_depth,
                                 float* final_T, int32_t* final_idx, int32_t* stop_pos, uint64_t* slot_ok,
                                 const TgsRasterOpts* opts, void* stream) {
  TGS_CHECK_ARG(camera_ok(cam), "bad camera");
  TGS_CHECK_ARG(splats && sorted_gid && tile_start && out_rgb && out_depth && final_T,
                "null pointer");
  const CamK k = make_camk(cam);
  const int T = k.TW * k.TH;
  TGS_CHECK_ARG(tile_start_len >= (int64_t)T + 1 + TGS_TILE_START_SCRATCH,
                "tile_start buffer shorter than tgs_tile_start_len(W, H) (the forward writes the scratch behind the starts)");
  const int grid = TGS_XCDS * tgs_xcd_slots(T);
#define TGS_LAUNCH_FWD(IDX, OK)                                                                          \
  hipLaunchKernelGGL((k_raster_fwd<IDX, OK>), dim3(grid), dim3(64), 0, (hipStream_t)stream, k, T, splats, \
                     sorted_gid, tile_start, out_rgb, out_depth, final_T, final_idx, tile_order,          \
                     (unsigned long long*)slot_ok, stop_pos)
  if (opt_or(opts, &TgsRasterOpts::k6_blocks, g_k6_blocks) && !slot_ok) {
    SplitRule sr;
    sr.factor = tile_order ? opt_or(opts, &TgsRasterOpts::k6_split, g_k6_split) : 0;
    sr.n_slots = grid;
    sr.heads = sr.factor > 0 ? min(grid, opt_or(opts, &TgsRasterOpts::k6_split_heads, g_k6_heads)) : 0;
    sr.floor = max(64, opt_or(opts, &TgsRasterOpts::k6_split_floor, g_k6_floor));
    const int blocks = grid + 3 * sr.heads;
    if (final_idx)
      hipLaunchKernelGGL(k_raster_fwd_blocks<true>, dim3(blocks), dim3(64), 0, (hipStream_t)stream, k, T, splats,
                         sorted_gid, tile_start, out_rgb, out_depth, final_T, final_idx, tile_order, stop_pos, sr);
    else
      hipLaunchKernelGGL(k_raster_fwd_blocks<false>, dim3(blocks), dim3(64), 0, (hipStream_t)stream, k, T, splats,
                         sorted_gid, tile_start, out_rgb, out_depth, final_T, final_idx, tile_order, stop_pos, sr);
    TGS_CHECK_LAUNCH();
    return TGS_OK;
  }
  if (final_idx) { if (slot_ok) TGS_LAUNCH_FWD(true, true); else TGS_LAUNCH_FWD(true, false); }
  else { if (slot_ok) TGS_LAUNCH_FWD(false, true); else TGS_LAUNCH_FWD(false, false); }
#undef TGS_LAUNCH_FWD
  TGS_CHECK_LAUNCH();
  return TGS_OK;
}

extern "C" int tgs_rasterize_depth_stats(const TgsCamera* cam, const float* splats, const int32_t* sorted_gid,
                                         const int32_t* tile_start, int64_t tile_start_len, const int32_t* tile_order,
                                         const float* out_depth, const float* final_T, const int32_t* stop_pos,
                                         float* depth_var, float* median_depth, int32_t* median_gid,
                                         const TgsRasterOpts* opts, void* stream) {
  TGS_CHECK_ARG(camera_ok(cam), "bad camera");
  TGS_CHECK_ARG(cam->W <= 255 * TGS_BLOCK && cam->H <= 255 * TGS_BLOCK, "image sides are limited to 4080 px (255 tiles)");
  TGS_CHECK_ARG(splats && sorted_gid && tile_start && out_depth && final_T && depth_var && median_depth, "null pointer");
  const CamK k = make_camk(cam);
  const int T = k.TW * k.TH;
  TGS_CHECK_ARG(tile_start_len >= (int64_t)T + 1 + TGS_TILE_START_SCRATCH,
                "tile_start buffer shorter than tgs_tile_start_len(W, H) (the buffer of the forward these lists were composited with)");
  const int grid = TGS_XCDS * tgs_xcd_slots(T);
  SplitRule sr;
  sr.factor = tile_order ? opt_or(opts, &TgsRasterOpts::k6_split, g_k6_split) : 0;
  sr.n_slots = grid;
  sr.heads = sr.factor > 0 ? min(grid, opt_or(opts, &TgsRasterOpts::k6_split_heads, g_k6_heads)) : 0;
  sr.floor = max(64, opt_or(opts, &TgsRasterOpts::k6_split_floor, g_k6_floor));
  DepthStatsOut o{depth_var, median_depth, median_gid};
  hipLaunchKernelGGL(k_raster_depth_stats, dim3(grid + 3 * sr.heads), dim3(64), 0, (hipStream_t)stream, k, T, splats,
                     sorted_gid, tile_start, out_depth, final_T, stop_pos, o, tile_order, sr);
  TGS_CHECK_LAUNCH();
  return TGS_OK;
}

static int rasterize_bwd_impl(const TgsCamera* cam, const float* splats,
                                 const int32_t* group_base, const int32_t* sorted_gid,
                                 int32_t* tile_start, int64_t tile_start_len, const int32_t* tile_order,
                                 const float* out_rgb, const float* out_depth,
                                 const float* final_T, const int32_t* stop_pos, const float* v_rgb,
                                 const float* v_depth, const float* v_alpha,
                                 const TgsLossSpec* loss, float* partials, float* tile_loss,
                                 int band, const uint64_t* slot_ok, const TgsRasterOpts* opts, void* stream) {
  TGS_CHECK_ARG(camera_ok(cam), "bad camera");
  TGS_CHECK_ARG(splats && group_base && sorted_gid && tile_start && out_rgb && out_depth &&
                final_T && partials, "null pointer");
  LossK lk;
  lk.on = 0; lk.gt_rgb = nullptr; lk.gt_depth = nullptr; lk.unc = nullptr;
  lk.l1w = lk.dw = lk.uw = 0.f; lk.eps = 1e-6f;
  if (loss) {
    lk.on = 1;
    lk.gt_rgb = (loss->l1_weight != 0.f) ? loss->gt_rgb : nullptr;
    lk.gt_depth = (loss->depth_weight != 0.f) ? loss->gt_depth : nullptr;
    lk.unc = loss->uncertainty;
    lk.l1w = loss->l1_weight; lk.dw = loss->depth_weight;
    lk.uw = loss->uncertainty_weight; lk.eps = loss->eps;
  }
  const CamK k = make_camk(cam);
  const int T = k.TW * k.TH;
  TGS_CHECK_ARG(tile_start_len >= (int64_t)T + 1 + TGS_TILE_START_SCRATCH,
                "tile_start buffer shorter than tgs_tile_start_len(W, H) (the backward keeps slot counters behind the starts)");
  int grid = TGS_XCDS * tgs_xcd_slots(T);
  if (band >= 0) {
    TGS_CHECK_ARG(tile_order, "a band launch needs the tile_order of tgs_bin_sort");
    TGS_CHECK_ARG(band < tgs_band_count(T), "band out of range");
    const int c = tgs_band_slots(T), s0 = band * c, s1 = min(s0 + c, tgs_xcd_slots(T));
    tile_order += (size_t)s0 * TGS_XCDS;
    grid = (s1 - s0) * TGS_XCDS;
  }
  if (opt_or(opts, &TgsRasterOpts::k7_front_to_back, g_k7_f2b) || slot_ok) {
    hipLaunchKernelGGL(k_raster_bwd_f2b, dim3(grid), dim3(64), 0, (hipStream_t)stream, k, T, splats,
                       group_base, sorted_gid, tile_start, out_rgb, out_depth, final_T,
                       v_rgb, v_depth, v_alpha, lk, partials, tile_loss, tile_order,
                       (const unsigned long long*)slot_ok);
  } else if (opt_or(opts, &TgsRasterOpts::k7_blocks, g_k7_blocks)) {
    TGS_CHECK_ARG(stop_pos, "stop_pos (written by tgs_rasterize_fwd) is required");
    hipLaunchKernelGGL(k_raster_bwd_blocks, dim3(grid), dim3(64), 0, (hipStream_t)stream, k, T, splats,
                       group_base, sorted_gid, tile_start, out_rgb, out_depth, final_T, stop_pos,
                       v_rgb, v_depth, v_alpha, lk, partials, tile_loss, tile_order);
  } else {
    TGS_CHECK_ARG(stop_pos, "stop_pos (written by tgs_rasterize_fwd) is required");
    QuadRule qf;
    qf.factor = band >= 0 ? 0 : opt_or(opts, &TgsRasterOpts::k7_quad, g_k7_quad);
    qf.min_walk = opt_or(opts, &TgsRasterOpts::k7_quad_min_walk, g_k7_quad_min);
    qf.scan_min = qf.factor > 0 ? g_k7_scan_min.get() : 0;
    qf.scan_heads = min(grid, g_k7_scan_heads.get());
    if (qf.scan_min > 0 && qf.scan_min < qf.min_walk) qf.scan_min = qf.min_walk;
    ScanSide* side = nullptr;
    if (qf.scan_min > 0 && qf.scan_heads > 0) {
      static const hipError_t scan_attr = hipFuncSetAttribute(reinterpret_cast<const void*>(k_raster_bwd_scan),
                                                              hipFuncAttributeMaxDynamicSharedMemorySize, SCAN_LDS_BYTES);
      TGS_CHECK_ARG(scan_attr == hipSuccess, "k_raster_bwd_scan: dynamic LDS size refused");
      hipStream_t ss = (hipStream_t)stream;
      if (g_k7_scan_side.get()) {
        side = &scan_side();
        TGS_CHECK_ARG(side->ok, "k_raster_bwd_scan: no side stream");
        TGS_HIP(hipEventRecord(side->fork, (hipStream_t)stream));
        TGS_HIP(hipStreamWaitEvent(side->s, side->fork, 0));
        ss = side->s;
      }
      hipLaunchKernelGGL(k_raster_bwd_scan, dim3(qf.scan_heads), dim3(1024), SCAN_LDS_BYTES, ss, k, T, splats,
                         group_base, sorted_gid, tile_start, out_rgb, out_depth, final_T, stop_pos,
                         v_rgb, v_depth, v_alpha, lk, partials, tile_order, qf);
      if (side) TGS_HIP(hipEventRecord(side->join, side->s));
    }
    hipLaunchKernelGGL(k_raster_bwd, dim3(grid), dim3(64), 0, (hipStream_t)stream, k, T, splats,
                       group_base, sorted_gid, tile_start, out_rgb, out_depth, final_T, stop_pos,
                       v_rgb, v_depth, v_alpha, lk, partials, tile_loss, tile_order, qf);
    if (qf.factor > 0) {
      TGS_CHECK_LAUNCH();
      hipLaunchKernelGGL(k_raster_bwd_quad, dim3(min(grid, 1280)), dim3(256), 0, (hipStream_t)stream, k, T, splats,
                         group_base, sorted_gid, tile_start, out_rgb, out_depth, final_T, stop_pos,
                         v_rgb, v_depth, v_alpha, lk, partials, tile_order, qf, grid);
    }
    if (side) TGS_HIP(hipStreamWaitEvent((hipStream_t)stream, side->join, 0));
  }
  TGS_CHECK_LAUNCH();
  return TGS_OK;
}

extern "C" int tgs_rasterize_bwd(const TgsCamera* cam, const float* splats,
                                 const int32_t* group_base, const int32_t* sorted_gid,
                                 int32_t* tile_start, int64_t tile_start_len, const int32_t* tile_order,
                                 const float* out_rgb, const float* out_depth,
                                 const float* final_T, const int32_t* stop_pos, const float* v_rgb,
                                 const float* v_depth, const float* v_alpha,
                                 const TgsLossSpec* loss, float* partials, float* tile_loss,
                                 const uint64_t* slot_ok, const TgsRasterOpts* opts, void* stream) {
  return rasterize_bwd_impl(cam, splats, group_base, sorted_gid, tile_start, tile_start_len, tile_order, out_rgb, out_depth, final_T, stop_pos, v_rgb, v_depth, v_alpha, loss, partials, tile_loss, -1, slot_ok, opts, stream);
}

extern "C" int tgs_rasterize_bwd_band(const TgsCamera* cam, const float* splats,
                                 const int32_t* group_base, const int32_t* sorted_gid,
                                 int32_t* tile_start, int64_t tile_start_len, const int32_t* tile_order,
                                 const float* out_rgb, const float* out_depth,
                                 const float* final_T, const int32_t* stop_pos, const float* v_rgb,
                                 const float* v_depth, const float* v_alpha,
                                 const TgsLossSpec* loss, float* partials, float* tile_loss,
                                 int band, const uint64_t* slot_ok, const TgsRasterOpts* opts, void* stream) {
  TGS_CHECK_ARG(band >= 0, "band < 0");
  return rasterize_bwd_impl(cam, splats, group_base, sorted_gid, tile_start, tile_start_len, tile_order, out_rgb, out_depth, final_T, stop_pos, v_rgb, v_depth, v_alpha, loss, partials, tile_loss, band, slot_ok, opts, stream);
}

extern "C" size_t tgs_slot_ok_len(int W, int H, int64_t capacity) {
  if (capacity < 0) capacity = 0;
  const size_t T = (size_t)((W + TGS_BLOCK - 1) / TGS_BLOCK) * (size_t)((H + TGS_BLOCK - 1) / TGS_BLOCK);
  return (size_t)(capacity >> 6) + T + 2;
}
```

touch_gs_amd/model.py:

```python
from __future__ import annotations

import collections
import os
import dataclasses
import math
from typing import Dict, Optional

import torch

from . import ops
from .camera import Camera
from .optim import FusedAdam, GaussianParams

DEPTH_LOSS_TYPES = ("DEPTH_UNCERTAINTY_WEIGHTED_LOSS", "SIMPLE_LOSS")


@dataclasses.dataclass
class ModelConfig:
    sh_degree: int = 3
    ssim_lambda: float = 0.2
    pipeline_ssim: bool = False
    pipeline_ssim_min_tiles: int = 0
    depth_loss_mult: float = 0.2
    depth_loss_type: str = "DEPTH_UNCERTAINTY_WEIGHTED_LOSS"
    uncertainty_weight: float = 1.0
    depth_eps: float = 1e-6
    mono_depth_mult: float = 0.0
    mono_depth_alpha_min: float = 0.5
    mono_depth_local_mult: float = 0.0
    mono_depth_patch_tiles: int = 8
    mono_depth_patch_min_fill: float = 0.25
    mono_depth_patch_min_var: float = 1e-3
    sh_degree_interval: int = 1000
    num_downscales: int = 0
    resolution_schedule: int = 250
    background_color: tuple = (0.0, 0.0, 0.0)
    lr_means: float = 1.6e-4
    lr_means_final: Optional[float] = 1.6e-6
    lr_means_max_steps: int = 30000
    lr_scales: float = 5e-3
    lr_quats: float = 1e-3
    lr_opac: float = 5e-2
    lr_sh_dc: float = 2.5e-3
    lr_sh_rest: float = 1.25e-4
    spatial_sort: bool = False
    resort_every_refines: int = 10
    balance_long_runs: bool = True
    long_run: int = 0

    def downscale_factor(self, step: int) -> int:
        if self.num_downscales <= 0 or self.resolution_schedule <= 0:
            return 1
        return 2 ** max(self.num_downscales - step // self.resolution_schedule, 0)

    def lr_means_at(self, step: int) -> float:
        if self.lr_means_final is None or self.lr_means_max_steps <= 0:
            return self.lr_means
        t = min(max(step, 0) / self.lr_means_max_steps, 1.0)
        return float(math.exp(math.log(self.lr_means) * (1 - t) + math.log(self.lr_means_final) * t))

    def lrs(self) -> Dict[str, float]:
        return dict(means=self.lr_means, log_scales=self.lr_scales, quats=self.lr_quats,
                    opac_logit=self.lr_opac, sh_dc=self.lr_sh_dc, sh_rest=self.lr_sh_rest)


@dataclasses.dataclass(frozen=True)
class Tuning:
    long_run: int = 0
    k6_split: Optional[int] = None
    k6_split_floor: Optional[int] = None
    k6_split_heads: Optional[int] = None

    def raster_opts(self):
        return ops.raster_opts(k6_split=self.k6_split, k6_split_floor=self.k6_split_floor, k6_split_heads=self.k6_split_heads)


@dataclasses.dataclass
class View:
    cam: Camera
    rgb: torch.Tensor
    depth: Optional[torch.Tensor] = None
    uncertainty: Optional[torch.Tensor] = None
    n_valid_depth: Optional[int] = None
    gt_depth: Optional[torch.Tensor] = None
    object_mask: Optional[torch.Tensor] = None
    mono_depth: Optional[torch.Tensor] = None

    def valid_count(self) -> int:
        if self.n_valid_depth is None:
            self.n_valid_depth = int((self.depth > 0).sum().item()) if self.depth is not None else 0
        return self.n_valid_depth

    def downscaled(self, d: int) -> "View":
        if d <= 1:
            return self
        cache = self.__dict__.setdefault("_downscaled", {})
        if d not in cache:
            H, W = self.rgb.shape[0] // d, self.rgb.shape[1] // d
            F = torch.nn.functional
            rgb = F.interpolate(self.rgb.permute(2, 0, 1)[None], size=(H, W), mode="bilinear", align_corners=False,
                                antialias=False)[0].permute(1, 2, 0).contiguous()
            near = lambda t: None if t is None else F.interpolate(t[None, None].float(), size=(H, W), mode="nearest")[0, 0].to(t.dtype).contiguous()
            cache[d] = View(cam=self.cam.downscaled(d), rgb=rgb, depth=near(self.depth), uncertainty=near(self.uncertainty),
                            gt_depth=near(self.gt_depth), object_mask=near(self.object_mask), mono_depth=near(self.mono_depth))
        return cache[d]


class DepthGaussianSplattingModel:
    list_hint = True
    LIST_HINT_AFTER = 16

    def __init__(self, config: ModelConfig, params: GaussianParams):
        self.config = config
        self.params = params
        self.step = 0
        self.populate_modules()

    def populate_modules(self):
        self.optimizer = FusedAdam(self.params, self.config.lrs())
        self.budget = ops.IntersectBudget()
        self._sync_budget = ops.IntersectBudget()
        self.fuse_adam = True
        self.dp_factored_sh = True
        self.front_prefetch = os.environ.get("TGS_FRONT_PREFETCH", "1") != "0"
        self._color_block = self._color_all = self._color_rows = None
        self.last = {}
        self.tuning = Tuning()
        self._tuned_cams = {}

    def tuned(self, cam: Camera, keep: bool = True) -> Camera:
        lr = self.tuning.long_run
        if lr == 0 or lr == cam.long_run:
            return cam
        hit = self._tuned_cams.get(id(cam))
        if hit is None or hit[0] is not cam or hit[1].long_run != lr:
            hit = (cam, dataclasses.replace(cam, long_run=lr))
            if keep:
                self._tuned_cams[id(cam)] = hit
        return hit[1]

    @property
    def num_points(self) -> int:
        return self.params.N

    def active_sh_degree(self, step: Optional[int] = None) -> int:
        c = self.config
        max_deg = int(round(math.sqrt(self.params.K))) - 1
        if c.sh_degree_interval <= 0:
            return min(c.sh_degree, max_deg)
        return min((self.step if step is None else step) // c.sh_degree_interval, c.sh_degree, max_deg)

    def get_outputs(self, cam: Camera, sh_degree: Optional[int] = None, depth_stats: bool = False) -> Dict[str, torch.Tensor]:
        p = self.params
        deg = self.active_sh_degree() if sh_degree is None else sh_degree
        budget = self.budget if self.budget.sync else self._sync_budget
        stats = ()
        if depth_stats:
            rgb, depth_acc, alpha, radii, *stats = ops.render(p.means, p.log_scales, p.quats, p.opac_logit, p.sh,
                                                              self.tuned(cam, keep=False), deg, budget=budget,
                                                              opts=self.tuning.raster_opts(), depth_stats=True)
        else:
            rgb, depth_acc, alpha, radii = ops.render(p.means, p.log_scales, p.quats, p.opac_logit, p.sh,
                                                      self.tuned(cam, keep=False), deg, budget=budget,
                                                      opts=self.tuning.raster_opts())
        depth = depth_acc / torch.clamp(alpha, min=1e-10)
        out = dict(rgb=rgb, depth=depth[..., None], accumulation=alpha[..., None],
                   depth_acc=depth_acc, alpha=alpha, radii=radii)
        if depth_stats:
            var, med, gid = stats
            out.update(median_depth=med[..., None], depth_var=var[..., None], depth_std=torch.sqrt(var)[..., None],
                       median_gid=gid)
        return out

    def depth_loss(self, depth_acc, alpha, view: View) -> torch.Tensor:
        c = self.config
        if c.depth_loss_type not in DEPTH_LOSS_TYPES:
            raise ValueError(c.depth_loss_type)
        m = view.depth > 0
        cnt = m.sum()
        dhat = depth_acc / torch.clamp(alpha, min=1e-10)
        r2 = (dhat - view.depth) ** 2
        if c.depth_loss_type == "DEPTH_UNCERTAINTY_WEIGHTED_LOSS" and view.uncertainty is not None:
            r2 = r2 / (c.uncertainty_weight * view.uncertainty + c.depth_eps)
        return torch.where(m, r2, torch.zeros_like(r2)).sum() / torch.clamp(cnt, min=1)

    def get_loss_dict(self, outputs, view: View) -> Dict[str, torch.Tensor]:
        c = self.config
        H, W = view.rgb.shape[:2]
        l1 = (outputs["rgb"] - view.rgb).abs().mean()
        loss = {"main_loss": (1 - c.ssim_lambda) * l1}
        if c.ssim_lambda > 0:
            loss["main_loss"] = loss["main_loss"] + c.ssim_lambda * (1 - _SSIM.apply(outputs["rgb"], view.rgb))
        if c.depth_loss_mult > 0 and view.depth is not None:
            loss["depth_loss"] = c.depth_loss_mult * self.depth_loss(outputs["depth_acc"], outputs["alpha"], view)
        if self.mono_depth_local_active(view):
            rho, rho_bar = ops.depth_correlation_local(outputs["depth_acc"], outputs["alpha"], view.mono_depth,
                                                       c.mono_depth_alpha_min, c.mono_depth_patch_tiles, self.patch_offset(),
                                                       c.mono_depth_patch_min_fill, c.mono_depth_patch_min_var)
            if c.mono_depth_mult > 0:
                loss["mono_depth_loss"] = c.mono_depth_mult * (1 - rho)
            loss["mono_depth_local_loss"] = c.mono_depth_local_mult * (1 - rho_bar)
        elif self.mono_depth_active(view):
            rho = ops.depth_correlation(outputs["depth_acc"], outputs["alpha"], view.mono_depth, c.mono_depth_alpha_min)
            loss["mono_depth_loss"] = c.mono_depth_mult * (1 - rho)
        return loss

    def mono_depth_active(self, view: View) -> bool:
        return self.config.mono_depth_mult > 0 and view.mono_depth is not None

    def mono_depth_local_active(self, view: View) -> bool:
        return self.config.mono_depth_local_mult > 0 and view.mono_depth is not None

    def patch_offset(self, step: Optional[int] = None):
        k = self.config.mono_depth_patch_tiles
        step = self.step if step is None else step
        return step % k, (step // k) % k

    @torch.no_grad()
    def get_metrics_dict(self, outputs, view: View) -> Dict[str, torch.Tensor]:
        mse = ((outputs["rgb"] - view.rgb) ** 2).mean()
        m = {"psnr": -10.0 * torch.log10(mse), "gaussian_count": torch.tensor(self.num_points)}
        if view.depth is not None:
            valid = view.depth > 0
            d = outputs["depth"][..., 0]
            m["depth_mse"] = ((d - view.depth)[valid] ** 2).mean() if valid.any() else torch.tensor(0.0)
        return m

    @torch.no_grad()
    def get_image_metrics_and_images(self, outputs, view: View):
        mse = ((outputs["rgb"] - view.rgb) ** 2).mean()
        ssim_sum, _ = ops.ssim_fwd_bwd(outputs["rgb"], view.rgb, want_grad=False)
        H, W = view.rgb.shape[:2]
        metrics = {"psnr": float(-10.0 * torch.log10(mse)), "ssim": float(ssim_sum) / (3 * H * W)}
        if view.depth is not None:
            valid = view.depth > 0
            d = outputs["depth"][..., 0]
            metrics["depth_mse"] = float(((d - view.depth)[valid] ** 2).mean()) if valid.any() else 0.0
            metrics["supervised_depth_mse"] = metrics["depth_mse"]
        if view.gt_depth is not None:
            d = outputs["depth"][..., 0]
            valid = view.gt_depth > 0
            metrics["gt_depth_mse"] = float(((d - view.gt_depth)[valid] ** 2).mean()) if valid.any() else 0.0
            if view.object_mask is not None:
                obj = valid & view.object_mask
                metrics["gt_object_depth_mse"] = float(((d - view.gt_depth)[obj] ** 2).mean()) if obj.any() else 0.0
        images = {"img": torch.cat([view.rgb, outputs["rgb"]], dim=1),
                  "depth": outputs["depth"], "accumulation": outputs["accumulation"]}
        if "median_depth" in outputs:
            dm = torch.where(outputs["median_gid"] >= 0, outputs["median_depth"][..., 0], outputs["depth"][..., 0])
            mse_of = lambda ref, m: float(((dm - ref)[m] ** 2).mean()) if m.any() else 0.0
            if view.depth is not None:
                metrics["median_depth_mse"] = mse_of(view.depth, view.depth > 0)
            if view.gt_depth is not None:
                valid = view.gt_depth > 0
                metrics["gt_depth_mse_median"] = mse_of(view.gt_depth, valid)
                if view.object_mask is not None:
                    metrics["gt_object_depth_mse_median"] = mse_of(view.gt_depth, valid & view.object_mask)
            images["median_depth"] = outputs["median_depth"]
            images["depth_std"] = outputs["depth_std"]
        return metrics, images

    def loss_spec(self, view: View) -> dict:
        c = self.config
        H, W = view.rgb.shape[:2]
        spec = dict(gt_rgb=view.rgb, l1_weight=(1 - c.ssim_lambda) / (3 * H * W))
        if c.depth_loss_mult > 0 and view.depth is not None:
            if c.depth_loss_type not in DEPTH_LOSS_TYPES:
                raise ValueError(c.depth_loss_type)
            cnt = max(view.valid_count(), 1)
            spec.update(gt_depth=view.depth, depth_weight=c.depth_loss_mult / cnt,
                        uncertainty=view.uncertainty if c.depth_loss_type == "DEPTH_UNCERTAINTY_WEIGHTED_LOSS" else None,
                        uncertainty_weight=c.uncertainty_weight, eps=c.depth_eps)
        return spec

    def forward_backward(self, view: View, want_v_xy: bool = False, fuse_adam: bool = False,
                         color_block: Optional[torch.Tensor] = None, begin_step: bool = True,
                         colors=None, prefetch=None, next_front=None):
        p, c, cam = self.params, self.config, self.tuned(view.cam)
        deg = self.active_sh_degree()
        H, W = cam.H, cam.W
        splats, radii, group_base, tile_start, sorted_gid, status = ops.project_bin_sort(
            cam, p.means, p.log_scales, p.quats, p.opac_logit, p.sh, deg, self.budget, want_radii=want_v_xy,
            colors=colors, next_front=next_front)
        guard = None if self.budget.sync else status
        rgb, depth_acc, fT, fidx = ops.rasterize_fwd(cam, splats, sorted_gid, tile_start, opts=self.tuning.raster_opts())
        v_img, ssim_sum = None, None
        mono_stats = v_depth = v_alpha = None
        patch_off = None
        if self.mono_depth_local_active(view):
            patch_off = self.patch_offset()
            mono_stats, v_depth, v_alpha = ops.depth_corr_local_fwd_bwd(
                depth_acc, fT, view.mono_depth, c.mono_depth_alpha_min, weight_global=max(c.mono_depth_mult, 0.0),
                weight_local=c.mono_depth_local_mult, patch_tiles=c.mono_depth_patch_tiles, offset=patch_off,
                min_fill=c.mono_depth_patch_min_fill, min_var_ratio=c.mono_depth_patch_min_var)
        elif self.mono_depth_active(view):
            mono_stats, v_depth, v_alpha = ops.depth_corr_fwd_bwd(depth_acc, fT, view.mono_depth, c.mono_depth_alpha_min,
                                                                  weight=c.mono_depth_mult)
        if (c.ssim_lambda > 0 and c.pipeline_ssim and cam.num_tiles >= c.pipeline_ssim_min_tiles and mono_stats is None
                and not torch.cuda.is_current_stream_capturing()):
            if getattr(self, "_side_stream", None) is None:
                self._side_stream = torch.cuda.Stream(device=rgb.device)
            partials, tile_loss, ssim_sum = ops.rasterize_bwd_ssim_pipelined(
                cam, splats, group_base, sorted_gid, tile_start, rgb, depth_acc, fT, view.rgb,
                -c.ssim_lambda / (3 * H * W), self.loss_spec(view), self._side_stream)
        else:
            if c.ssim_lambda > 0:
                ssim_sum, v_img = ops.ssim_fwd_bwd(rgb, view.rgb, weight=-c.ssim_lambda / (3 * H * W), reduce=False)
            partials, tile_loss = ops.rasterize_bwd(cam, splats, group_base, sorted_gid, tile_start, rgb,
                                                    depth_acc, fT, v_rgb=v_img, v_depth=v_depth, v_alpha=v_alpha,
                                                    loss=self.loss_spec(view), want_tile_loss=True)
        if fuse_adam:
            v_xy = self.optimizer.backward_and_step(cam, deg, splats, group_base, partials, want_v_xy,
                                                    begin=begin_step, guard=guard, prefetch=prefetch)
        elif color_block is not None:
            if isinstance(color_block, (list, tuple)):
                rows, blocks = color_block
                v_xy = torch.empty(p.N, 2, dtype=torch.float32, device=p.flat.device) if want_v_xy else None
                out4 = p.grad_views()[:4]

                def backward_chunk(c, cam=cam, deg=deg, splats=splats, group_base=group_base, partials=partials,
                                   guard=guard, v_xy=v_xy):
                    ops.project_bwd_color(cam, p.means, p.log_scales, p.quats, p.opac_logit, p.sh, deg, splats,
                                          group_base, partials, out4, blocks[c], guard=guard, rows=rows[c], v_xy=v_xy)
                self._backward_chunk = backward_chunk
            else:
                v_xy = ops.project_bwd_color(cam, p.means, p.log_scales, p.quats, p.opac_logit, p.sh, deg, splats,
                                             group_base, partials, p.grad_views()[:4], color_block, want_v_xy,
                                             guard=guard)
        else:
            v_xy = ops.project_bwd(cam, p.means, p.log_scales, p.quats, p.opac_logit, p.sh, deg, splats,
                                   group_base, partials, out=p.grad_views(), want_v_xy=want_v_xy, guard=guard)[5]
        self.last = dict(rgb=rgb, depth_acc=depth_acc, final_T=fT, splats=splats, v_xy=v_xy, radii=radii,
                         tile_loss=tile_loss, ssim_sum=ssim_sum, status=status, guard=guard, view=view)
        if mono_stats is not None:
            self.last["mono_stats"] = mono_stats
        if patch_off is not None:
            self.last["mono_patch_offset"] = patch_off
        return tile_loss, ssim_sum

    def loss_from(self, tile_loss, ssim_sum, view: View, mono_stats=None) -> Dict[str, torch.Tensor]:
        c = self.config
        H, W = view.rgb.shape[:2]
        t = tile_loss.sum(0)
        main = t[0]
        if ssim_sum is not None:
            main = main + c.ssim_lambda * (1 - ssim_sum.sum() / (3 * H * W))
        out = {"main_loss": main, "depth_loss": t[1]}
        if mono_stats is None and self.last.get("tile_loss") is tile_loss:
            mono_stats = self.last.get("mono_stats")
        if mono_stats is not None:
            if mono_stats.numel() == 8 or c.mono_depth_mult > 0:
                out["mono_depth_loss"] = mono_stats[7]
            if mono_stats.numel() == 16:
                out["mono_depth_local_loss"] = mono_stats[11]
        return out

    def spatial_sort(self) -> torch.Tensor:
        from .optim import balanced_order
        hits = None
        cams = list(getattr(self, "_recent_cams", {}).values()) if self.config.balance_long_runs else []
        if os.environ.get("TGS_BALANCE_LONG_RUNS", "1") == "0":
            cams = []
        if cams:
            p, hits = self.params, 0
            for cam in cams:
                sp = ops.project_fwd(cam, p.means, p.log_scales, p.quats, p.opac_logit, None, -1)
                rect = sp[:, 10].contiguous().view(torch.int32)
                hits = hits + ((rect >> 16) & 255) * ((rect >> 24) & 255)
            dp = getattr(self, "_dp", None)
            if dp is not None and dp.active:
                import torch.distributed as dist
                n_cams = torch.tensor([len(cams)], dtype=torch.int64, device=hits.device)
                hits = hits.to(torch.int64)
                dist.all_reduce(hits, op=dist.ReduceOp.SUM)
                dist.all_reduce(n_cams, op=dist.ReduceOp.SUM)
                hits = (hits + int(n_cams) - 1) // int(n_cams)
            else:
                hits = (hits + len(cams) - 1) // len(cams)
        if hits is not None:
            if self.config.long_run > 0:
                self.tuning = Tuning(long_run=self.config.long_run)
            elif float(hits[hits > 32].sum()) / max(float(hits.sum()), 1.0) > 0.3:
                self.tuning = Tuning(long_run=8, k6_split=1, k6_split_floor=128, k6_split_heads=2048)
            else:
                self.tuning = Tuning(long_run=32)
        long_run = self.tuning.long_run or 32
        perm = balanced_order(self.params.means, hits, long_run=long_run)
        self.params.permute_(perm, self.optimizer.exp_avg, self.optimizer.exp_avg_sq)
        density = getattr(self, "density", None)
        if density is not None:
            density.grad_norm_sum = density.grad_norm_sum[perm]
            density.vis_count = density.vis_count[perm]
            density.max_radius = density.max_radius[perm]
        self._graphs = {}
        self._tuned_cams = {}
        self._prefetch_ready = None
        self._refines_since_sort = 0
        return perm

    def enable_densification(self, cfg=None):
        from .densify import DensifyConfig, DensityController
        self.density = DensityController(cfg or DensifyConfig(), self.params.N, self.params.flat.device)

    def enable_speculative_budget(self, capacity: int = 0, max_in_flight: int = 4) -> None:
        self.budget = ops.IntersectBudget(capacity=capacity, sync=False, speculative=True)
        self._pending = collections.deque()
        self._max_in_flight = max_in_flight
        self._pinned = []
        self._dp_status = None
        self._dp = None
        self._seen_longest, self._good_frames = 0, 0

    def _speculative_track(self, view: View, distributed: bool = False) -> None:
        host = self._pinned.pop() if self._pinned else torch.zeros(7, dtype=torch.int32).pin_memory()
        host[:4].copy_(self.budget.last_status4, non_blocking=True)
        if distributed:
            host[4:6].copy_(self._dp_status, non_blocking=True)
        peer = getattr(self._dp, "peer", None) if distributed else None
        if peer is not None:
            host[6:].copy_(peer.err_word, non_blocking=True)
        else:
            host[6] = 0
        ev = torch.cuda.Event()
        ev.record()
        self._pending.append((view, host, ev))
        if distributed:
            if len(self._pending) > self._max_in_flight:
                self._speculative_poll(block=True, only_one=True)
        else:
            self._speculative_poll(block=len(self._pending) > self._max_in_flight)

    def _speculative_poll(self, block: bool = False, drain: bool = False, only_one: bool = False) -> None:
        while self._pending and (drain or block or (not only_one and self._dp is None and self._pending[0][2].query())):
            view, host, ev = self._pending[0]
            ev.synchronize()
            block = False
            if int(host[6]) != 0:
                self._dp.peer.raise_if(int(host[6]))
            if int(host[5] if self._dp is not None else host[1]) == 0:
                self._pending.popleft()
                self._seen_need = max(getattr(self, "_seen_need", 0), int(host[2]), int(host[0]))
                self._seen_longest = max(self._seen_longest, int(host[3]))
                self._good_frames += 1
                dens = getattr(self, "density", None)
                need_frames = max(self.LIST_HINT_AFTER, dens.cfg.num_train_data if dens is not None else 0,
                                  len(getattr(self, "_recent_cams", ())))
                if self.list_hint and self._good_frames >= need_frames:
                    self.budget.max_list_hint = max(self.budget.max_list_hint, int(1.5 * self._seen_longest) + 64)
                self._pinned.append(host)
                if only_one:
                    return
                continue
            torch.cuda.synchronize()
            redo = list(self._pending)
            self._pending.clear()
            need = max(int(h[0]) for _, h, _ in redo)
            self.budget.capacity = max(self.budget.capacity, int(need * self.budget.growth) + 1024)
            self._seen_longest = max([self._seen_longest] + [int(h[3]) for _, h, _ in redo])
            self.budget.max_list_hint, self._good_frames = -1, 0
            self.budget.sticky.zero_()
            self._prefetch_ready = None
            self.optimizer.t -= len(redo)
            self.step -= len(redo)
# ... 224 lines not shown
```

touch_gs_amd/ops.py:

```python
from __future__ import annotations

import ctypes as C
import math
from typing import Optional, Tuple

import torch

from . import _lib
from ._lib import PARTIAL_FLOATS, SPLAT_FLOATS, check, ptr
from .camera import Camera


def _stream():
    return C.c_void_p(torch.cuda.current_stream().cuda_stream)


import os as _os
SLOT_OK = _os.environ.get("TGS_SLOT_OK", "0") == "1"


def _f32c(t: Optional[torch.Tensor]):
    if t is None:
        return None
    if t.dtype != torch.float32:
# ... 143 lines not shown
    def __init__(self, cam: Camera, N: int, cap: int, want_radii: bool, dev):
        lib = _lib.load()
        T = cam.num_tiles
        self.N, self.cap, self.cam = N, cap, cam
        self.splats = torch.empty(max(N, 1), SPLAT_FLOATS, dtype=torch.float32, device=dev)[:N]
        self.radii = torch.empty(N, dtype=torch.int32, device=dev) if want_radii else None
        self.group_base = torch.empty(max(lib.tgs_num_groups(N), 1), dtype=torch.int32, device=dev)
        self.tile_start = torch.empty(T + 1 + 512, dtype=torch.int32, device=dev)[:T + 1]
        nc = lib.tgs_tile_counter_len(cam.W, cam.H)
        counters = torch.empty(nc + 4, dtype=torch.int32, device=dev)
        self.tile_cursor, self.status, self.status4 = counters[:nc], counters[nc:nc + 2], counters[nc:]
        self.tile_start.tile_order = torch.empty(lib.tgs_tile_order_len(cam.W, cam.H), dtype=torch.int32, device=dev)
        self.tile_start.slot_ok = None
        self.sorted_gid = torch.empty(max(cap, 1), dtype=torch.int32, device=dev)
        self.scratch = torch.empty(lib.tgs_sort_scratch_bytes(cap), dtype=torch.uint8, device=dev)
        self.cleared = False


def project_bin_sort(cam: Camera, means, log_scales, quats, opac_logit, sh, sh_deg: int,
                     budget: Optional[IntersectBudget] = None, want_radii: bool = False,
                     colors: Optional[ColorPrefetch] = None, next_front: Optional["FrontBuffers"] = None):
    lib = _lib.load()
    budget = budget or _default_budget
    N = means.shape[0]
    dev = means.device
    cs = cam.c_struct()
    sh_stride = sh.shape[1] if sh is not None else 0
    cap = budget.initial(N)
    fb = colors.front if (colors is not None and sh is not None and N > 0 and colors.front_issued) else None
    if fb is not None:
        colors.front, colors.front_issued = None, False
        if (fb.N != N or fb.cap != cap or fb.cam is not cam or colors.front_budget is not budget
                or (want_radii and fb.radii is None)):
            fb = None
    from_front = fb is not None
    tag_holder = colors
    if colors is not None and not colors.colors_valid:
        colors = None
    if fb is None:
        fb = FrontBuffers(cam, N, cap, want_radii, dev)
    splats, radii, group_base, tile_start = fb.splats, fb.radii, fb.group_base, fb.tile_start
    tile_cursor, status, status4, tile_order = fb.tile_cursor, fb.status, fb.status4, fb.tile_start.tile_order
    sorted_gid, scratch = fb.sorted_gid, fb.scratch
    while True:
        if from_front:
            nf = next_front if (_SIDE_CLEAR and next_front is not None and not next_front.cleared and next_front is not fb and
                                lib.tgs_front_can_clear_next(N, next_front.cam.W, next_front.cam.H)) else None
            ncs = nf.cam.c_struct() if nf is not None else None
            check(lib.tgs_project_bin_sort_front(C.byref(cs), N, ptr(means), ptr(log_scales), ptr(quats), ptr(opac_logit),
                                                 ptr(sh), sh_stride, sh_deg, ptr(splats), ptr(radii), ptr(group_base),
                                                 ptr(tile_start), _tile_start_len(tile_start), ptr(tile_cursor), ptr(sorted_gid),
                                                 ptr(tile_order), cap, ptr(scratch), ptr(status), ptr(budget.sticky_word(dev)),
                                                 budget.list_hint(), ptr(tag_holder.tag_word), tag_holder.tag,
                                                 C.byref(ncs) if nf is not None else None,
                                                 ptr(nf.tile_cursor) if nf is not None else None,
                                                 ptr(nf.status) if nf is not None else None, _stream()),
                  "tgs_project_bin_sort_front")
            if nf is not None:
                nf.cleared = True
            from_front = False
        elif colors is None or sh is None:
            check(lib.tgs_project_bin_sort(C.byref(cs), N, ptr(means), ptr(log_scales), ptr(quats), ptr(opac_logit),
                                           ptr(sh), sh_stride, sh_deg if sh is not None else -1, ptr(splats),
                                           ptr(radii), ptr(group_base), ptr(tile_start), _tile_start_len(tile_start),
                                           ptr(tile_cursor), ptr(sorted_gid), ptr(tile_order), cap, ptr(scratch), ptr(status),
                                           ptr(budget.sticky_word(dev)), budget.list_hint(), _stream()),
                  "tgs_project_bin_sort")
        else:
            check(lib.tgs_project_bin_sort_colors(C.byref(cs), N, ptr(means), ptr(log_scales), ptr(quats),
                                                  ptr(opac_logit), ptr(sh), sh_stride, sh_deg, ptr(splats),
                                                  ptr(radii), ptr(group_base), ptr(tile_start), _tile_start_len(tile_start),
                                                  ptr(tile_cursor), ptr(sorted_gid), ptr(tile_order), cap, ptr(scratch), ptr(status),
                                                  ptr(budget.sticky_word(dev)), budget.list_hint(), ptr(colors.colors),
                                                  ptr(colors.tag_word), colors.tag, _stream()),
                  "tgs_project_bin_sort_colors")
        budget.last_status = status
        budget.last_status4 = status4
        if not budget.sync:
            break
        n, ovf, need, budget.last_longest = status4.tolist()
        budget.last_n, budget.last_need = n, max(n, need)
        if not ovf:
            break
        cap = int(n * budget.growth) + 1024
        budget.capacity = cap
        sorted_gid = torch.empty(max(cap, 1), dtype=torch.int32, device=dev)
        scratch = torch.empty(lib.tgs_sort_scratch_bytes(cap), dtype=torch.uint8, device=dev)
    return splats, radii, group_base, tile_start, sorted_gid, status


def _tile_start_len(tile_start) -> int:
    return tile_start.untyped_storage().nbytes() // 4 - tile_start.storage_offset()


def raster_opts(k6_blocks=None, k6_split=None, k7_front_to_back=None, k7_quad=None, k7_quad_min_walk=None, k7_blocks=None,
                k6_split_floor=None, k6_split_heads=None):
    f = lambda v: -1 if v is None else int(v)
    return _lib.TgsRasterOpts(f(k6_blocks), f(k6_split), f(k7_front_to_back), f(k7_quad), f(k7_quad_min_walk), f(k7_blocks),
                              f(k6_split_floor), f(k6_split_heads))


def _check_tile_start(tile_start, T: int) -> None:
    have = _tile_start_len(tile_start)
    if have < T + 1 + 512:
        raise ValueError(f"tile_start must be (a view of) a buffer of T + 513 = {T + 513} int32 (got room for {have}): "
                         "pass the tensor ops.bin_sort / ops.project_bin_sort returned, not a copy")


def rasterize_fwd(cam: Camera, splats, sorted_gid, tile_start, want_idx: bool = False, want_stop: bool = True, opts=None):
    lib = _lib.load()
    dev = splats.device
    H, W = cam.H, cam.W
    _check_tile_start(tile_start, cam.num_tiles)
    rgb = torch.empty(H, W, 3, dtype=torch.float32, device=dev)
    depth = torch.empty(H, W, dtype=torch.float32, device=dev)
    fT = torch.empty(H, W, dtype=torch.float32, device=dev)
    fidx = torch.empty(H, W, dtype=torch.int32, device=dev) if want_idx else None
    stop = torch.empty(H, W, dtype=torch.int32, device=dev) if want_stop else None
    fT.stop_pos = stop
    cs = cam.c_struct()
    slot_ok = None
    if SLOT_OK and hasattr(tile_start, "slot_ok"):
        slot_ok = torch.empty(4 * lib.tgs_slot_ok_len(W, H, sorted_gid.shape[0]), dtype=torch.int64, device=dev)
        tile_start.slot_ok = slot_ok
    check(lib.tgs_rasterize_fwd(C.byref(cs), ptr(splats), ptr(sorted_gid), ptr(tile_start), _tile_start_len(tile_start),
                                ptr(getattr(tile_start, "tile_order", None)), ptr(rgb),
                                ptr(depth), ptr(fT), ptr(fidx), ptr(stop), ptr(slot_ok),
                                C.byref(opts) if opts is not None else None, _stream()), "tgs_rasterize_fwd")
    return rgb, depth, fT, fidx


def rasterize_depth_stats(cam: Camera, splats, sorted_gid, tile_start, depth_acc, final_T, want_gid: bool = False, opts=None):
    lib = _lib.load()
    dev = splats.device
    H, W = cam.H, cam.W
    _check_tile_start(tile_start, cam.num_tiles)
    depth_acc, fT = _f32c(depth_acc.detach()), _f32c(final_T.detach())
    if tuple(depth_acc.shape) != (H, W) or tuple(fT.shape) != (H, W):
        raise ValueError(f"depth_acc / final_T must be [{H},{W}]")
    stop = getattr(final_T, "stop_pos", None)
    var = torch.empty(H, W, dtype=torch.float32, device=dev)
    med = torch.empty(H, W, dtype=torch.float32, device=dev)
    gid = torch.empty(H, W, dtype=torch.int32, device=dev) if want_gid else None
    cs = cam.c_struct()
    check(lib.tgs_rasterize_depth_stats(C.byref(cs), ptr(splats), ptr(sorted_gid), ptr(tile_start), _tile_start_len(tile_start),
                                        ptr(getattr(tile_start, "tile_order", None)), ptr(depth_acc), ptr(fT), ptr(stop),
                                        ptr(var), ptr(med), ptr(gid), C.byref(opts) if opts is not None else None,
                                        _stream()), "tgs_rasterize_depth_stats")
    return var, med, gid


def rasterize_bwd(cam: Camera, splats, group_base, sorted_gid, tile_start, rgb, depth, fT,
                  v_rgb=None, v_depth=None, v_alpha=None, loss: Optional[dict] = None,
                  want_tile_loss: bool = False, stop_pos=None, partials=None, opts=None):
    lib = _lib.load()
    dev = splats.device
    _check_tile_start(tile_start, cam.num_tiles)
    if partials is None:
        partials = torch.empty(sorted_gid.shape[0], PARTIAL_FLOATS, dtype=torch.float32, device=dev)
    tile_loss = torch.empty(cam.num_tiles, 2, dtype=torch.float32, device=dev) if want_tile_loss else None
    cs = cam.c_struct()
    ls = None
    keep = []
    if loss is not None:
        ls = _loss_spec_struct(loss, keep)
    v_rgb, v_depth, v_alpha = _f32c(v_rgb), _f32c(v_depth), _f32c(v_alpha)
    check(lib.tgs_rasterize_bwd(C.byref(cs), ptr(splats), ptr(group_base), ptr(sorted_gid),
                                ptr(tile_start), _tile_start_len(tile_start), ptr(getattr(tile_start, "tile_order", None)),
                                ptr(rgb), ptr(depth), ptr(fT), ptr(_stop_pos_of(fT, stop_pos)),
                                ptr(v_rgb), ptr(v_depth), ptr(v_alpha),
                                C.byref(ls) if ls is not None else None, ptr(partials),
                                ptr(tile_loss), ptr(getattr(tile_start, "slot_ok", None)),
                                C.byref(opts) if opts is not None else None, _stream()), "tgs_rasterize_bwd")
    return partials, tile_loss


def set_raster_variant(k6_blocks: Optional[bool] = None, k7_front_to_back: Optional[bool] = None) -> int:
    f = lambda v: -1 if v is None else int(bool(v))
    return _lib.load().tgs_set_raster_variant(f(k6_blocks), f(k7_front_to_back))


def set_k6_split_shape(floor: Optional[int] = None, heads: Optional[int] = None):
    r = _lib.load().tgs_set_k6_split_shape(-1 if floor is None else int(floor), -1 if heads is None else int(heads))
    return r & 0xffff, r >> 16


def set_long_run(tiles: Optional[int] = None) -> int:
    return _lib.load().tgs_set_long_run(-1 if tiles is None else int(tiles))


def set_k6_split(factor: Optional[int] = None) -> int:
    return _lib.load().tgs_set_k6_split(-1 if factor is None else int(factor))


def set_k7_quad(factor: Optional[int] = None, min_walk: Optional[int] = None):
    r = _lib.load().tgs_set_k7_quad(-1 if factor is None else int(factor), -1 if min_walk is None else int(min_walk))
    return r & 255, r >> 8


def set_k7_scan(min_walk: Optional[int] = None, heads: Optional[int] = None):
    r = _lib.load().tgs_set_k7_scan(-1 if min_walk is None else int(min_walk), -1 if heads is None else int(heads))
    return r & 0xffff, r >> 16


def _stop_pos_of(fT, stop_pos=None):
    sp = stop_pos if stop_pos is not None else getattr(fT, "stop_pos", None)
    if sp is None:
        raise RuntimeError("rasterize_bwd needs the forward's stop positions: pass the final_T tensor that "
                           "rasterize_fwd returned (it carries .stop_pos) or stop_pos=...")
    return sp


def _loss_spec_struct(loss, keep):
    ls = _lib.TgsLossSpec()
    for k in ("gt_rgb", "gt_depth", "uncertainty"):
        t = _f32c(loss.get(k))
        keep.append(t)
        setattr(ls, k, ptr(t))
    ls.l1_weight = float(loss.get("l1_weight", 0.0))
    ls.depth_weight = float(loss.get("depth_weight", 0.0))
    ls.uncertainty_weight = float(loss.get("uncertainty_weight", 1.0))
    ls.eps = float(loss.get("eps", 1e-6))
    return ls


def band_rows(cam: Camera):
    lib = _lib.load()
    TW = cam.tiles[0]
    out = []
    t0, t1 = C.c_int(), C.c_int()
    for b in range(lib.tgs_num_bands(cam.W, cam.H)):
        check(lib.tgs_band_tiles(cam.W, cam.H, b, C.byref(t0), C.byref(t1)), "tgs_band_tiles")
        if t1.value > t0.value:
            out.append([b, 16 * (t0.value // TW), min(16 * ((t1.value - 1) // TW + 1), cam.H)])
    for i, r in enumerate(out):
        r += [r[1] if i else 0, out[i + 1][1] if i + 1 < len(out) else cam.H]
    return [tuple(r) for r in out]


def rasterize_bwd_ssim_pipelined(cam: Camera, splats, group_base, sorted_gid, tile_start, rgb, depth, fT, gt_rgb,
                                 ssim_weight: float, loss: Optional[dict], side_stream, want_tile_loss: bool = True):
    lib = _lib.load()
    dev = splats.device
    H, W = cam.H, cam.W
    order = getattr(tile_start, "tile_order", None)
    if order is None:
        raise ValueError("the band launches need tile_start.tile_order (ops.bin_sort / project_bin_sort)")
    bands = band_rows(cam)
    rgb, gt_rgb = _f32c(rgb), _f32c(gt_rgb)
    partials = torch.empty(sorted_gid.shape[0], PARTIAL_FLOATS, dtype=torch.float32, device=dev)
    tile_loss = torch.empty(cam.num_tiles, 2, dtype=torch.float32, device=dev) if want_tile_loss else None
    v_img = torch.empty_like(rgb)
    scratch = torch.empty(9 * H * W, dtype=torch.float32, device=dev)
    n_p = ((W + 63) // 64) * ((max(y1 - y0 for _, y0, y1, _, _ in bands) + 10) // 12 + 2)
    bp = torch.empty(len(bands), n_p, dtype=torch.float32, device=dev)
    keep = []
    ls = _loss_spec_struct(loss, keep) if loss is not None else None
    cs = cam.c_struct()
    main = torch.cuda.current_stream(dev)
    ready = torch.cuda.Event()
    ready.record(main)
    side_stream.wait_event(ready)
    for t in (v_img, scratch, bp, rgb, gt_rgb):
        t.record_stream(side_stream)
    done = []
    with torch.cuda.stream(side_stream):
        for i, (b, y0, y1, c0, c1) in enumerate(bands):
            check(lib.tgs_ssim_fwd_bwd_rows(W, H, ptr(rgb), ptr(gt_rgb), C.c_float(ssim_weight), ptr(bp[i]), n_p,
                                            ptr(v_img), ptr(scratch), y0, y1, c0, c1, _stream()),
                  "tgs_ssim_fwd_bwd_rows")
            ev = torch.cuda.Event()
            ev.record(side_stream)
            done.append(ev)
    for (b, *_), ev in zip(bands, done):
        main.wait_event(ev)
        check(lib.tgs_rasterize_bwd_band(C.byref(cs), ptr(splats), ptr(group_base), ptr(sorted_gid), ptr(tile_start),
                                         _tile_start_len(tile_start), ptr(order), ptr(rgb), ptr(depth), ptr(fT),
                                         ptr(_stop_pos_of(fT)), ptr(v_img), None, None,
                                         C.byref(ls) if ls is not None else None, ptr(partials), ptr(tile_loss),
                                         b, ptr(getattr(tile_start, "slot_ok", None)), None, _stream()), "tgs_rasterize_bwd_band")
    return partials, tile_loss, bp


def reduce_partials(cam: Camera, splats, group_base, partials):
    lib = _lib.load()
    N = splats.shape[0]
    v_splats = torch.empty(N, SPLAT_FLOATS, dtype=torch.float32, device=splats.device)
    cs = cam.c_struct()
    check(lib.tgs_reduce_partials(N, ptr(splats), ptr(group_base), C.byref(cs), ptr(partials),
                                  ptr(v_splats), _stream()), "tgs_reduce_partials")
    return v_splats


def project_bwd(cam: Camera, means, log_scales, quats, opac_logit, sh, sh_deg, splats,
                group_base=None, partials=None, v_splats=None, out=None, want_v_xy=False, guard=None):
    lib = _lib.load()
    N = means.shape[0]
    dev = means.device
    e = lambda *s: torch.empty(*s, dtype=torch.float32, device=dev)
    if out is None:
        out = (e(N, 3), e(N, 3), e(N, 4), e(N), torch.empty_like(sh) if sh is not None else None)
    v_means, v_ls, v_q, v_ol, v_sh = out
    v_xy = e(N, 2) if want_v_xy else None
    cs = cam.c_struct()
    sh_stride = sh.shape[1] if sh is not None else 0
    check(lib.tgs_project_bwd(C.byref(cs), N, ptr(means), ptr(log_scales), ptr(quats), ptr(opac_logit),
                              ptr(sh), sh_stride, sh_deg if sh is not None else -1, ptr(splats),
                              ptr(group_base), ptr(partials), ptr(v_splats), ptr(v_means), ptr(v_ls),
                              ptr(v_q), ptr(v_ol), ptr(v_sh), ptr(v_xy), ptr(guard), _stream()), "tgs_project_bwd")
    return v_means, v_ls, v_q, v_ol, v_sh, v_xy


def project_bwd_color(cam: Camera, means, log_scales, quats, opac_logit, sh, sh_deg, splats, group_base,
                      partials, out, v_color, want_v_xy=False, guard=None, rows=None, v_xy=None):
    lib = _lib.load()
    N = means.shape[0]
    b, e = (0, N) if rows is None else rows
    if v_color.numel() != 3 * (e - b) + 4 or v_color.dtype != torch.float32:
        raise ValueError("v_color must be a float32 tensor of 3*rows+4 elements")
    v_means, v_ls, v_q, v_ol = out
    if v_xy is None and want_v_xy:
        if rows is not None:
            raise ValueError("a row-range call writes into the caller's v_xy [N,2]")
        v_xy = torch.empty(N, 2, dtype=torch.float32, device=means.device)
    cs = cam.c_struct()
    check(lib.tgs_project_bwd_color_rows(C.byref(cs), N, b, e, ptr(means), ptr(log_scales), ptr(quats), ptr(opac_logit),
                                         ptr(sh), sh.shape[1], sh_deg, ptr(splats), ptr(group_base), ptr(partials),
# ... 90 lines not shown
        (dirs,) = ctx.saved_tensors
        v = torch.empty(ctx.shape, dtype=torch.float32, device=dirs.device)
        check(lib.tgs_sh_bwd(ctx.shape[0], ctx.deg, ctx.shape[1], ptr(dirs), ptr(_f32c(v_colors)), ptr(v), _stream()),
              "tgs_sh_bwd")
        return None, None, v


def spherical_harmonics(degrees_to_use: int, viewdirs: torch.Tensor, coeffs: torch.Tensor):
    return _SphericalHarmonics.apply(degrees_to_use, viewdirs, coeffs)


def record_xy(splats: torch.Tensor) -> torch.Tensor:
    r = splats[:, 10].contiguous().view(torch.int32)
    org = torch.stack([r & 255, (r >> 8) & 255], 1).to(torch.float32) * 16.0
    return (splats[:, 0:2] + org).contiguous()


class _ProjectGaussians(torch.autograd.Function):
    @staticmethod
    def forward(ctx, means3d, scales, glob_scale, quats, cam):
        means3d, quats = _f32c(means3d), _f32c(quats)
        log_scales = torch.log(_f32c(scales))
        N = means3d.shape[0]
        zero = torch.zeros(N, dtype=torch.float32, device=means3d.device)
        cam = Camera(cam.viewmat, cam.fx, cam.fy, cam.cx, cam.cy, cam.W, cam.H, cam.near,
                     cam.pix_center, cam.bg, float(glob_scale))
        splats, radii = project_fwd(cam, means3d, log_scales, quats, zero, None, -1, want_radii=True)
        ctx.cam = cam
        ctx.save_for_backward(means3d, log_scales, quats, zero, splats)
        xys = record_xy(splats)
        depths = splats[:, 2].contiguous()
        conics = splats[:, 4:7].contiguous()
        ctx.mark_non_differentiable(radii)
        return xys, depths, radii, conics

    @staticmethod
    def backward(ctx, v_xys, v_depths, _v_radii, v_conics):
        means3d, log_scales, quats, zero, splats = ctx.saved_tensors
        N = means3d.shape[0]
        v_splats = torch.zeros(N, SPLAT_FLOATS, dtype=torch.float32, device=means3d.device)
        if v_xys is not None:
            v_splats[:, 0:2] = v_xys
        if v_depths is not None:
            v_splats[:, 2] = v_depths
        if v_conics is not None:
            v_splats[:, 4:7] = v_conics
        v_means, v_ls, v_q, _, _, _ = project_bwd(ctx.cam, means3d, log_scales, quats, zero, None, -1,
                                                  splats, v_splats=v_splats)
        v_scales = v_ls / torch.exp(log_scales)
        return v_means, v_scales, None, v_q, None


def project_gaussians(means3d, scales, glob_scale, quats, viewmat, fx, fy, cx, cy, img_height,
                      img_width, block_width: int = 16, clip_thresh: float = 0.01):
    if block_width != 16:
        raise ValueError("only 16x16 tiles are supported (SURVEY App. B.0)")
    cam = Camera(viewmat, fx, fy, cx, cy, img_width, img_height, near=clip_thresh)
    xys, depths, radii, conics = _ProjectGaussians.apply(means3d, scales, glob_scale, quats, cam)
    with torch.no_grad():
        tw, th = cam.tiles
        r = radii.to(torch.float32)
        x0 = torch.clamp(((xys[:, 0] - r) / 16).to(torch.int32), 0, tw)
        x1 = torch.clamp(((xys[:, 0] + r) / 16).to(torch.int32) + 1, 0, tw)
        y0 = torch.clamp(((xys[:, 1] - r) / 16).to(torch.int32), 0, th)
        y1 = torch.clamp(((xys[:, 1] + r) / 16).to(torch.int32) + 1, 0, th)
        num_tiles_hit = torch.where(radii > 0, (x1 - x0) * (y1 - y0), torch.zeros_like(x0))
        q = quats / quats.norm(dim=-1, keepdim=True)
        w, x, y, z = q.unbind(-1)
        R = torch.stack([1 - 2 * (y * y + z * z), 2 * (x * y - w * z), 2 * (x * z + w * y),
                         2 * (x * y + w * z), 1 - 2 * (x * x + z * z), 2 * (y * z - w * x),
                         2 * (x * z - w * y), 2 * (y * z + w * x), 1 - 2 * (x * x + y * y)], -1).view(-1, 3, 3)
        M = R * (scales * glob_scale)[:, None, :]
        S = M @ M.transpose(1, 2)
        cov3d = torch.stack([S[:, 0, 0], S[:, 0, 1], S[:, 0, 2], S[:, 1, 1], S[:, 1, 2], S[:, 2, 2]], -1)
        comp = torch.ones_like(depths)
    return xys, depths, radii, conics, comp, num_tiles_hit, cov3d


class _RasterizeGaussians(torch.autograd.Function):
    @staticmethod
    def forward(ctx, xys, depths, radii, conics, colors, opacity, cam, budget):
        N = xys.shape[0]
        dev = xys.device
        op = opacity.reshape(N, 1).to(torch.float32)
        tw, th = cam.tiles
        r = radii.to(torch.float32)
        xf, yf = xys[:, 0].to(torch.float32), xys[:, 1].to(torch.float32)
        x0 = torch.clamp(((xf - r) * 0.0625).to(torch.int64), 0, tw)
        x1 = torch.clamp(((xf + r) * 0.0625).to(torch.int64) + 1, 0, tw)
        y0 = torch.clamp(((yf - r) * 0.0625).to(torch.int64), 0, th)
        y1 = torch.clamp(((yf + r) * 0.0625).to(torch.int64) + 1, 0, th)
        vis = (radii > 0) & (x1 > x0) & (y1 > y0)
        packed = torch.where(vis, x0 | (y0 << 8) | ((x1 - x0) << 16) | ((y1 - y0) << 24), torch.zeros_like(x0))
        packed = torch.where(packed >= 2 ** 31, packed - 2 ** 32, packed).to(torch.int32)
        org = torch.stack([x0, y0], 1).to(torch.float32) * 16.0
        org = torch.where(vis[:, None], org, torch.zeros_like(org))
        splats = torch.cat([xys.to(torch.float32) - org, depths.reshape(N, 1).to(torch.float32), op,
                            conics.to(torch.float32), colors.to(torch.float32),
                            packed.reshape(N, 1).view(torch.float32),
                            torch.zeros(N, 1, dtype=torch.float32, device=dev)], dim=1).contiguous()
        group_base, tile_start, sorted_gid, _ = bin_sort(cam, splats, budget)
        rgb, depth, fT, fidx = rasterize_fwd(cam, splats, sorted_gid, tile_start)
        ctx.cam = cam
        ctx.opacity_shape = opacity.shape
        ctx.save_for_backward(splats, group_base, tile_start, sorted_gid, rgb, depth, fT, fT.stop_pos)
        return rgb, 1.0 - fT, depth

    @staticmethod
    def backward(ctx, v_rgb, v_alpha, v_depth):
        splats, group_base, tile_start, sorted_gid, rgb, depth, fT, stop = ctx.saved_tensors
        cam = ctx.cam
        partials, _ = rasterize_bwd(cam, splats, group_base, sorted_gid, tile_start, rgb, depth, fT,
                                    v_rgb, v_depth, v_alpha, stop_pos=stop)
        v = reduce_partials(cam, splats, group_base, partials)
        v_xys, v_depths = v[:, 0:2].contiguous(), v[:, 2].contiguous()
        v_op = v[:, 3].contiguous().reshape(ctx.opacity_shape)
        v_conics, v_colors = v[:, 4:7].contiguous(), v[:, 7:10].contiguous()
        return v_xys, v_depths, None, v_conics, v_colors, v_op, None, None


def rasterize_gaussians(xys, depths, radii, conics, num_tiles_hit, colors, opacity, img_height,
                        img_width, block_width: int = 16, background=None, return_alpha: bool = False,
                        return_depth: bool = False, budget: Optional[IntersectBudget] = None):
    if block_width != 16:
        raise ValueError("only 16x16 tiles are supported (SURVEY App. B.0)")
    if colors.shape[-1] != 3:
        raise ValueError("colors must be [N,3]")
    bg = (0.0, 0.0, 0.0) if background is None else tuple(float(b) for b in background.detach().cpu().tolist())
    eye = [[1, 0, 0, 0], [0, 1, 0, 0], [0, 0, 1, 0], [0, 0, 0, 1]]
    cam = Camera(eye, 1.0, 1.0, 0.0, 0.0, img_width, img_height, bg=bg)
    rgb, alpha, depth = _RasterizeGaussians.apply(xys, depths, radii, conics, colors, opacity, cam, budget)
    out = (rgb,)
    if return_alpha:
        out += (alpha,)
    if return_depth:
        out += (depth,)
    return out[0] if len(out) == 1 else out


def ssim_fwd_bwd(img, gt, weight: float = 1.0, want_grad: bool = True, reduce: bool = True):
    lib = _lib.load()
    img, gt = _f32c(img), _f32c(gt)
    H, W = img.shape[0], img.shape[1]
    dev = img.device
    nb = ((H + 15) // 16) * ((W + 15) // 16)
    bp = torch.empty(nb, dtype=torch.float32, device=dev)
    v_img = torch.empty_like(img) if want_grad else None
    scratch = torch.empty(9 * H * W, dtype=torch.float32, device=dev) if want_grad else None
    check(lib.tgs_ssim_fwd_bwd(W, H, ptr(img), ptr(gt), C.c_float(weight), ptr(bp), ptr(v_img),
                               ptr(scratch), _stream()), "tgs_ssim_fwd_bwd")
    return (bp.sum() if reduce else bp), v_img


def depth_corr_fwd_bwd(depth_acc, final_T, mono, alpha_min: float = 0.5, weight: float = 1.0, want_grad: bool = True):
    lib = _lib.load()
    depth_acc, final_T, mono = _f32c(depth_acc.detach()), _f32c(final_T.detach()), _f32c(mono)
    if depth_acc.dim() != 2 or depth_acc.shape != final_T.shape or depth_acc.shape != mono.shape:
        raise ValueError(f"depth_acc, final_T and mono must be [H,W] alike, got {tuple(depth_acc.shape)}, "
                         f"{tuple(final_T.shape)}, {tuple(mono.shape)}")
    H, W = depth_acc.shape
    dev = depth_acc.device
    tiles = torch.empty(((H + 15) // 16) * ((W + 15) // 16), 8, dtype=torch.float32, device=dev)
    stats = torch.empty(8, dtype=torch.float32, device=dev)
    v_depth = torch.empty(H, W, dtype=torch.float32, device=dev) if want_grad else None
    v_alpha = torch.empty(H, W, dtype=torch.float32, device=dev) if want_grad else None
    check(lib.tgs_depth_corr_fwd_bwd(W, H, ptr(depth_acc), ptr(final_T), ptr(mono), C.c_float(alpha_min), C.c_float(weight),
                                     ptr(tiles), ptr(stats), ptr(v_depth), ptr(v_alpha), _stream()), "tgs_depth_corr_fwd_bwd")
    return stats, v_depth, v_alpha


class _DepthCorrelation(torch.autograd.Function):
    @staticmethod
    def forward(ctx, depth_acc, alpha, mono, alpha_min):
        stats, v_depth, v_alpha = depth_corr_fwd_bwd(depth_acc, 1.0 - alpha.detach(), mono, alpha_min, weight=-1.0)
        ctx.save_for_backward(v_depth, v_alpha)
        return stats[6].clone()

    @staticmethod
    def backward(ctx, g):
        v_depth, v_alpha = ctx.saved_tensors
        return g * v_depth, g * v_alpha, None, None


def depth_correlation(depth_acc, alpha, mono, alpha_min: float = 0.5):
    return _DepthCorrelation.apply(depth_acc, alpha, mono, alpha_min)


def depth_corr_patch_min_count(patch_tiles: int, min_fill: float) -> int:
    return max(2, math.ceil(min_fill * (16 * patch_tiles) ** 2))


def depth_corr_local_fwd_bwd(depth_acc, final_T, mono, alpha_min: float = 0.5, weight_global: float = 1.0,
                             weight_local: float = 1.0, patch_tiles: int = 8, offset=(0, 0), min_fill: float = 0.25,
                             min_var_ratio: float = 1e-3, want_grad: bool = True, return_patches: bool = False):
    lib = _lib.load()
    depth_acc, final_T, mono = _f32c(depth_acc.detach()), _f32c(final_T.detach()), _f32c(mono)
    if depth_acc.dim() != 2 or depth_acc.shape != final_T.shape or depth_acc.shape != mono.shape:
        raise ValueError(f"depth_acc, final_T and mono must be [H,W] alike, got {tuple(depth_acc.shape)}, "
                         f"{tuple(final_T.shape)}, {tuple(mono.shape)}")
    k, (off_x, off_y) = int(patch_tiles), (int(o) for o in offset)
    if not 1 <= k <= 16 or not (0 <= off_x < k and 0 <= off_y < k):
        raise ValueError(f"patch_tiles must be 1...16 and the offset in [0, patch_tiles), got {patch_tiles}, {tuple(offset)}")
    H, W = depth_acc.shape
    dev = depth_acc.device
    TW, TH = (W + 15) // 16, (H + 15) // 16
    PW, PH = (TW + off_x + k - 1) // k, (TH + off_y + k - 1) // k
    tiles = torch.empty(TW * TH, 8, dtype=torch.float32, device=dev)
    patches = torch.empty(PH, PW, 8, dtype=torch.float32, device=dev)
    stats = torch.empty(16, dtype=torch.float32, device=dev)
    v_depth = torch.empty(H, W, dtype=torch.float32, device=dev) if want_grad else None
    v_alpha = torch.empty(H, W, dtype=torch.float32, device=dev) if want_grad else None
    check(lib.tgs_depth_corr_local_fwd_bwd(W, H, ptr(depth_acc), ptr(final_T), ptr(mono), C.c_float(alpha_min),
                                           C.c_float(weight_global), C.c_float(weight_local), k, off_x, off_y,
                                           depth_corr_patch_min_count(k, min_fill), C.c_float(min_var_ratio), ptr(tiles),
                                           ptr(patches), ptr(stats), ptr(v_depth), ptr(v_alpha), _stream()),
          "tgs_depth_corr_local_fwd_bwd")
    return (stats, v_depth, v_alpha, patches) if return_patches else (stats, v_depth, v_alpha)


class _DepthCorrelationLocal(torch.autograd.Function):
    @staticmethod
    def forward(ctx, depth_acc, alpha, mono, alpha_min, patch_tiles, offset, min_fill, min_var_ratio):
        fT = 1.0 - alpha.detach()
        kw = dict(patch_tiles=patch_tiles, offset=offset, min_fill=min_fill, min_var_ratio=min_var_ratio)
        stats, gd, ga = depth_corr_local_fwd_bwd(depth_acc, fT, mono, alpha_min, -1.0, 0.0, **kw)
        _, ld, la = depth_corr_local_fwd_bwd(depth_acc, fT, mono, alpha_min, 0.0, -1.0, **kw)
        ctx.save_for_backward(gd, ga, ld, la)
        return stats[6].clone(), stats[10].clone()

    @staticmethod
    def backward(ctx, g_rho, g_bar):
        gd, ga, ld, la = ctx.saved_tensors
        return g_rho * gd + g_bar * ld, g_rho * ga + g_bar * la, None, None, None, None, None, None


def depth_correlation_local(depth_acc, alpha, mono, alpha_min: float = 0.5, patch_tiles: int = 8, offset=(0, 0),
                            min_fill: float = 0.25, min_var_ratio: float = 1e-3):
    return _DepthCorrelationLocal.apply(depth_acc, alpha, mono, alpha_min, patch_tiles, tuple(offset), min_fill, min_var_ratio)
```

Before: 994.7 iters/s.

## Fuse SSIM backward filter into rasterize-backward prologue with planar adjoint layout

The SSIM forward kernel can now write its per-pixel adjoint terms into a padded planar buffer. The rasterizer backward kernel gains a templated prologue that applies the separable Gaussian filter per tile and forms the SSIM image gradient in registers, so the separate SSIM backward kernel and the v_rgb write and read are dropped. The fused path is on by default when K7 runs in its default form. It adds shared-memory filter work and register pressure to the raster backward kernel, and chain-bound tiles still write v_rgb for the handoff path.

```diff
diff --git a/include/tgs.h b/include/tgs.h
--- a/include/tgs.h
+++ b/include/tgs.h
@@ -137,6 +137,16 @@
                       const TgsLossSpec* loss , float* partials, float* tile_loss,
                       const uint64_t* slot_ok , const TgsRasterOpts* opts ,
                       void* stream);
+
+int tgs_rasterize_bwd_ssim(const TgsCamera* cam , const float* splats,
+                           const int32_t* group_base, const int32_t* sorted_gid,
+                           int32_t* tile_start, int64_t tile_start_len, const int32_t* tile_order ,
+                           const float* out_rgb, const float* out_depth, const float* final_T,
+                           const int32_t* stop_pos, float* v_rgb, const float* v_depth, const float* v_alpha,
+                           const TgsLossSpec* loss , float* partials, float* tile_loss,
+                           const float* ssim_adj, float ssim_weight,
+                           const TgsRasterOpts* opts , void* stream);
+int tgs_k7_is_default_form(const TgsRasterOpts* opts );
 
 int tgs_rasterize_bwd_band(const TgsCamera* cam , const float* splats,
                       const int32_t* group_base, const int32_t* sorted_gid,
@@ -250,6 +260,10 @@
                           float* block_partials, int n_partials, float* v_img, float* scratch,
                           int y0, int y1, int count_y0, int count_y1, void* stream);
 
+size_t tgs_ssim_adj_len(int W, int H);
+int tgs_ssim_fwd_adjoint(int W, int H, const float* img, const float* gt, float* block_partials,
+                         float* adj, void* stream);
+
 int tgs_depth_corr_fwd_bwd(int W, int H, const float* out_depth, const float* final_T, const float* mono,
                            float alpha_min, float weight, float* tile_moments, float* stats,
                            float* v_depth , float* v_alpha , void* stream);
diff --git a/touch_gs_amd/_lib.py b/touch_gs_amd/_lib.py
--- a/touch_gs_amd/_lib.py
+++ b/touch_gs_amd/_lib.py
@@ -70,6 +70,9 @@
     "tgs_set_k6_split_shape": (C.c_int, [_I, _I]),
     "tgs_slot_ok_len": (C.c_size_t, [_I, _I, C.c_int64]),
     "tgs_rasterize_bwd": (C.c_int, [C.POINTER(TgsCamera)] + [_P] * 4 + [C.c_int64] + [_P] * 8 + [C.POINTER(TgsLossSpec), _P, _P, _P, C.POINTER(TgsRasterOpts), _P]),
+    "tgs_rasterize_bwd_ssim": (C.c_int, [C.POINTER(TgsCamera)] + [_P] * 4 + [C.c_int64] + [_P] * 8 + [C.POINTER(TgsLossSpec), _P, _P, _P, C.c_float,
+                                         C.POINTER(TgsRasterOpts), _P]),
+    "tgs_k7_is_default_form": (C.c_int, [C.POINTER(TgsRasterOpts)]),
     "tgs_rasterize_bwd_band": (C.c_int, [C.POINTER(TgsCamera)] + [_P] * 4 + [C.c_int64] + [_P] * 8 + [C.POINTER(TgsLossSpec), _P, _P, _I, _P, C.POINTER(TgsRasterOpts), _P]),
     "tgs_reduce_partials": (C.c_int, [_I, _P, _P, C.POINTER(TgsCamera), _P, _P, _P]),
     "tgs_project_bwd": (C.c_int, [C.POINTER(TgsCamera), _I, _P, _P, _P, _P, _P, _I, _I] + [_P] * 12),
@@ -96,6 +99,8 @@
     "tgs_adam_step": (C.c_int, [_I, _I, _P, _P, _P, _P, C.POINTER(TgsAdamSpec), C.c_float, C.c_int64, C.c_int64, _P, _P]),
     "tgs_ssim_fwd_bwd": (C.c_int, [_I, _I, _P, _P, C.c_float, _P, _P, _P, _P]),
     "tgs_ssim_fwd_bwd_rows": (C.c_int, [_I, _I, _P, _P, C.c_float, _P, _I, _P, _P, _I, _I, _I, _I, _P]),
+    "tgs_ssim_adj_len": (C.c_size_t, [_I, _I]),
+    "tgs_ssim_fwd_adjoint": (C.c_int, [_I, _I, _P, _P, _P, _P, _P]),
     "tgs_depth_corr_fwd_bwd": (C.c_int, [_I, _I, _P, _P, _P, C.c_float, C.c_float, _P, _P, _P, _P, _P]),
     "tgs_depth_corr_local_fwd_bwd": (C.c_int, [_I, _I, _P, _P, _P, C.c_float, C.c_float, C.c_float, _I, _I, _I, _I, C.c_float,
                                               _P, _P, _P, _P, _P, _P]),
diff --git a/touch_gs_amd/csrc/imgloss.hip b/touch_gs_amd/csrc/imgloss.hip
--- a/touch_gs_amd/csrc/imgloss.hip
+++ b/touch_gs_amd/csrc/imgloss.hip
@@ -1,18 +1,16 @@
 #include <math.h>
 #include <stdlib.h>
 #include "tgs_common.h"
+#include "tgs_ssim.h"
 
 namespace {
 
-constexpr int WIN = 11, HALO = 5;
+constexpr int WIN = TGS_SSIM_WIN, HALO = TGS_SSIM_HALO;
 struct Win { float g[WIN]; };
 #ifdef TGS_SSIM_SGPR_WINDOW
 #define WK(k) win.g[k]
 #else
-__device__ constexpr float WGT[WIN] = {0x1.0d956cp-10f, 0x1.f1fe02p-8f, 0x1.26eb18p-5f, 0x1.bff0fep-4f, 0x1.b43c4p-3f,
-                                       0x1.10656p-2f, 0x1.b43c4p-3f, 0x1.bff0fep-4f, 0x1.26eb18p-5f, 0x1.f1fe02p-8f,
-                                       0x1.0d956cp-10f};
-#define WK(k) WGT[k]
+#define WK(k) TGS_SSIM_WGT[k]
 #endif
 
 #ifndef TGS_SSIM_DMA
@@ -98,6 +96,7 @@
   }
 };
 
+template <bool PLANAR>
 __global__ __launch_bounds__(NTH) __attribute__((amdgpu_waves_per_eu(4, 8))) void k_ssim_fwd(int W, int H, Win win,
                                                   const float* __restrict__ img,
                                                   const float* __restrict__ gt,
@@ -181,10 +180,12 @@
             const float dm_ds12 = 2.f * n1 * id1 * id2;
             const float dm_ds11 = -m * id2;
             const float dm_dmu1 = 2.f * mu2 * n2 * id1 * id2 - m * 2.f * mu1 * id1;
-            float* o3 = adj + (((size_t)gy * W + gx) * 3 + c) * 3;
+            const size_t st = PLANAR ? tgs_ssim_adj_plane(W, H) : 1;
+            float* o3 = PLANAR ? adj + 3 * c * st + (size_t)(gy + HALO) * tgs_ssim_adj_pitch(W) + gx + HALO
+                               : adj + (((size_t)gy * W + gx) * 3 + c) * 3;
             o3[0] = dm_dmu1 - 2.f * mu1 * dm_ds11 - mu2 * dm_ds12;
-            o3[1] = dm_ds11;
-            o3[2] = dm_ds12;
+            o3[st] = dm_ds11;
+            o3[2 * st] = dm_ds12;
           }
         }
       }
@@ -261,7 +262,7 @@
         }
         if (gx < W) {
           const size_t pidx = (size_t)gy * W * 3 + (size_t)x0 * 3 + tid;
-          v_img[pidx] = weight * (o0 + 2.f * img[pidx] * o1 + gt[pidx] * o2);
+          v_img[pidx] = tgs_ssim_combine(weight, o0, o1, o2, img[pidx], gt[pidx]);
         }
       }
     }
@@ -387,7 +388,7 @@
 
 static int ssim_impl(int W, int H, const float* img, const float* gt, float weight,
                      float* block_partials, int n_partials, float* v_img, float* scratch,
-                     int y0, int y1, int c0, int c1, void* stream) {
+                     int y0, int y1, int c0, int c1, void* stream, float* planar_adj = nullptr) {
   TGS_CHECK_ARG(W > 0 && H > 0, "bad image size");
   TGS_CHECK_ARG(img && gt && block_partials, "null pointer");
   TGS_CHECK_ARG(!v_img || scratch, "gradient needs scratch");
@@ -412,7 +413,8 @@
     TGS_CHECK_LAUNCH();
     return TGS_OK;
   }
-  const int f0 = v_img ? max(0, y0 - HALO) : y0, f1 = v_img ? min(H, y1 + HALO) : y1;
+  const bool want_adj = v_img || planar_adj;
+  const int f0 = want_adj ? max(0, y0 - HALO) : y0, f1 = want_adj ? min(H, y1 + HALO) : y1;
   const int rows = f1 - f0;
   if (rows <= 0) return TGS_OK;
   const int sx = (W + SW - 1) / SW;
@@ -424,8 +426,12 @@
   const int SEG = seg_rows(nblk);
   const dim3 block(NTH);
   hipStream_t s = (hipStream_t)stream;
-  hipLaunchKernelGGL(k_ssim_fwd, dim3(sx, (rows + SEG - 1) / SEG, 1), block, 0, s, W, H, win, img, gt,
-                     v_img ? scratch : nullptr, block_partials, n_partials, nblk, f0, f1, c0, c1);
+  if (planar_adj)
+    hipLaunchKernelGGL(k_ssim_fwd<true>, dim3(sx, (rows + SEG - 1) / SEG, 1), block, 0, s, W, H, win, img, gt,
+                       planar_adj, block_partials, n_partials, nblk, f0, f1, c0, c1);
+  else
+    hipLaunchKernelGGL(k_ssim_fwd<false>, dim3(sx, (rows + SEG - 1) / SEG, 1), block, 0, s, W, H, win, img, gt,
+                       v_img ? scratch : nullptr, block_partials, n_partials, nblk, f0, f1, c0, c1);
   TGS_CHECK_LAUNCH();
   if (v_img && y1 > y0) {
     hipLaunchKernelGGL(k_ssim_bwd, dim3(sx, (y1 - y0 + SEG - 1) / SEG, 1), block, 0, s, W, H, win, weight, img, gt,
@@ -449,3 +455,15 @@
   return ssim_impl(W, H, img, gt, weight, block_partials, n_partials, v_img, scratch, y0, y1, count_y0,
                    count_y1, stream);
 }
+
+extern "C" size_t tgs_ssim_adj_len(int W, int H) {
+  if (W <= 0 || H <= 0) return 0;
+  return 9 * tgs_ssim_adj_plane(W, H);
+}
+
+extern "C" int tgs_ssim_fwd_adjoint(int W, int H, const float* img, const float* gt, float* block_partials,
+                                    float* adj, void* stream) {
+  TGS_CHECK_ARG(adj && ((uintptr_t)adj & 15) == 0, "adj is null or not 16-byte aligned");
+  return ssim_impl(W, H, img, gt, 0.f, block_partials, ((W + 15) / 16) * ((H + 15) / 16), nullptr, nullptr,
+                   0, H, 0, H, stream, adj);
+}
diff --git a/touch_gs_amd/csrc/raster.hip b/touch_gs_amd/csrc/raster.hip
--- a/touch_gs_amd/csrc/raster.hip
+++ b/touch_gs_amd/csrc/raster.hip
@@ -1,6 +1,7 @@
 #include <stdlib.h>
 #include <type_traits>
 #include "tgs_common.h"
+#include "tgs_ssim.h"
 
 namespace {
 
@@ -975,6 +976,8 @@
 #ifndef TGS_K7_PAIR
 #define TGS_K7_PAIR 0
 #endif
+struct SsimK { const float* adj; const float* gt; float* v_out; float weight; int pitch; size_t plane; };
+template <bool SSIM>
 #if TGS_K7_RECPF
 __attribute__((amdgpu_waves_per_eu(4, 8)))
 #endif
@@ -985,14 +988,18 @@
     const float* __restrict__ final_T, const int32_t* __restrict__ stop_pos, const float* __restrict__ v_rgb,
     const float* __restrict__ v_depth, const float* __restrict__ v_alpha, LossK loss,
     float* __restrict__ partials, float* __restrict__ tile_loss,
-    const int32_t* __restrict__ tile_order, QuadRule quad) {
+    const int32_t* __restrict__ tile_order, QuadRule quad, SsimK ssim) {
   if (blockIdx.x == 0 && threadIdx.x < TGS_WALK_WORDS && quad.factor > 0)
     frame_scratch(tile_start)[TGS_SLOTCTR_AT(T_total, threadIdx.x)] = 0;
+  __shared__ float4 recs[64 * 3];
+  __shared__ float4 sums[64 * 4];
+  constexpr int RED_RS = 68;
+  constexpr int RED_ROWS = 8;
+  __shared__ float4 red4[(TGS_K7_PAIR ? 2 : 1) * RED_ROWS * RED_RS / 4];
   const int tile = tile_order ? tile_order[blockIdx.x] : xcd_tile(blockIdx.x, T_total);
   if (tile >= T_total) return;
   const int lane = threadIdx.x;
   const int ty = tile / cam.TW, tx = tile - ty * cam.TW;
-  const PixConst pc = make_pix_const(lane);
   const int start = tile_start[tile], end = tile_start[tile + 1];
   const int n = end - start;
 
@@ -1000,18 +1007,61 @@
   float vCr[4], vCg[4], vCb[4], vD[4], SX[4];
   int lim[4];
   float l_l1 = 0.f, l_dep = 0.f;
+  [[maybe_unused]] int qlim_s[4] = {0, 0, 0, 0};
+  [[maybe_unused]] int tmax_s = 0;
+  [[maybe_unused]] bool handoff_s = false;
+  [[maybe_unused]] float vI[3][4];
+  if constexpr (SSIM) {
+#pragma unroll
+    for (int k = 0; k < 4; k++) {
+      const int px = tx * TGS_BLOCK + 8 * (k & 1) + (lane & 7);
+      const int py = ty * TGS_BLOCK + 8 * (k >> 1) + (lane >> 3);
+      lim[k] = (px < cam.W && py < cam.H) ? min(stop_pos[(size_t)py * cam.W + px], n) : 0;
+      vI[0][k] = vI[1][k] = vI[2][k] = 0.f;
+    }
+    if (n > 0) {
+#pragma unroll
+      for (int k = 0; k < 4; k++) qlim_s[k] = wave_minmax_i<true>(lim[k]);
+      tmax_s = max(max(qlim_s[0], qlim_s[1]), max(qlim_s[2], qlim_s[3]));
+      handoff_s = tmax_s > quad.min_walk && frame_is_chain_bound(tile_start, T_total, quad);
+    }
+    if (tmax_s > 0) {
+      static_assert(TGS_SSIM_HBUF * sizeof(float) <= sizeof(sums), "the filter's scratch aliases sums");
+      const float* win = ssim.adj + (size_t)(ty * TGS_BLOCK) * ssim.pitch + tx * TGS_BLOCK;
+      const float* rgb2 = out_rgb;
+      asm volatile("" : "+s"(rgb2));
+      tgs_ssim_bwd_tile(win, ssim.pitch, ssim.plane, lane, reinterpret_cast<float*>(sums), [&](auto CC, const float (&o)[4][3]) {
+        constexpr int c = decltype(CC)::value;
+#pragma unroll
+        for (int k = 0; k < 4; k++) {
+          const int px = tx * TGS_BLOCK + 8 * (k & 1) + (lane & 7);
+          const int py = ty * TGS_BLOCK + 8 * (k >> 1) + (lane >> 3);
+          if (px < cam.W && py < cam.H) {
+            const size_t p = ((size_t)py * cam.W + px) * 3 + c;
+            float v = tgs_ssim_combine(ssim.weight, o[k][0], o[k][1], o[k][2], rgb2[p], ssim.gt[p]);
+            asm volatile("" : "+v"(v));
+            vI[c][k] = v;
+            if (handoff_s) ssim.v_out[p] = v;
+          }
+        }
+      });
+    }
+  }
+  const PixConst pc = make_pix_const(lane);
 #pragma unroll
   for (int k = 0; k < 4; k++) {
     const int px = tx * TGS_BLOCK + 8 * (k & 1) + (lane & 7);
     const int py = ty * TGS_BLOCK + 8 * (k >> 1) + (lane >> 3);
-    lim[k] = 0; vCr[k] = vCg[k] = vCb[k] = vD[k] = SX[k] = 0.f;
+    if constexpr (!SSIM) lim[k] = 0;
+    vCr[k] = vCg[k] = vCb[k] = vD[k] = SX[k] = 0.f;
     if (px < cam.W && py < cam.H) {
       const size_t p = (size_t)py * cam.W + px;
       const float Tf = final_T[p];
       T[k] = Tf;
-      lim[k] = min(stop_pos[p], n);
+      if constexpr (!SSIM) lim[k] = min(stop_pos[p], n);
       float vA = v_alpha ? v_alpha[p] : 0.f;
-      if (v_rgb) { vCr[k] = v_rgb[3 * p]; vCg[k] = v_rgb[3 * p + 1]; vCb[k] = v_rgb[3 * p + 2]; }
+      if constexpr (SSIM) { vCr[k] = vI[0][k]; vCg[k] = vI[1][k]; vCb[k] = vI[2][k]; }
+      else if (v_rgb) { vCr[k] = v_rgb[3 * p]; vCg[k] = v_rgb[3 * p + 1]; vCb[k] = v_rgb[3 * p + 2]; }
       if (v_depth) vD[k] = v_depth[p];
       if (loss.on) {
         if (loss.gt_rgb) {
@@ -1049,10 +1099,15 @@
   }
   if (n == 0) return;
   int qlim[4];
-#pragma unroll
-  for (int k = 0; k < 4; k++) qlim[k] = wave_minmax_i<true>(lim[k]);
+  if constexpr (SSIM) {
+#pragma unroll
+    for (int k = 0; k < 4; k++) qlim[k] = qlim_s[k];
+  } else {
+#pragma unroll
+    for (int k = 0; k < 4; k++) qlim[k] = wave_minmax_i<true>(lim[k]);
+  }
   const int tmax = max(max(qlim[0], qlim[1]), max(qlim[2], qlim[3]));
-  if (tmax > quad.min_walk && frame_is_chain_bound(tile_start, T_total, quad)) return;
+  if (SSIM ? handoff_s : (tmax > quad.min_walk && frame_is_chain_bound(tile_start, T_total, quad))) return;
   const float4 z4 = make_float4(0.f, 0.f, 0.f, 0.f);
   for (int i = start + tmax + lane; i < end; i += 64) {
     const int gid = sorted_gid[i];
@@ -1062,11 +1117,6 @@
   }
   if (tmax == 0) return;
 
-  __shared__ float4 recs[64 * 3];
-  __shared__ float4 sums[64 * 4];
-  constexpr int RED_RS = 68;
-  constexpr int RED_ROWS = 8;
-  __shared__ float4 red4[(TGS_K7_PAIR ? 2 : 1) * RED_ROWS * RED_RS / 4];
   float* red = reinterpret_cast<float*>(red4);
   const int red_c = lane & 15;
   const int red_part = (lane >> 4) ^ ((red_c >= 4 && red_c < 12) ? 1 : 0);
@@ -2206,6 +2256,11 @@
   return TGS_OK;
 }
 
+extern "C" int tgs_k7_is_default_form(const TgsRasterOpts* opts) {
+  if (opt_or(opts, &TgsRasterOpts::k7_front_to_back, g_k7_f2b) || opt_or(opts, &TgsRasterOpts::k7_blocks, g_k7_blocks)) return 0;
+  return !(opt_or(opts, &TgsRasterOpts::k7_quad, g_k7_quad) > 0 && g_k7_scan_min.get() > 0);
+}
+
 static int rasterize_bwd_impl(const TgsCamera* cam, const float* splats,
                                  const int32_t* group_base, const int32_t* sorted_gid,
                                  int32_t* tile_start, int64_t tile_start_len, const int32_t* tile_order,
@@ -2213,10 +2268,17 @@
                                  const float* final_T, const int32_t* stop_pos, const float* v_rgb,
                                  const float* v_depth, const float* v_alpha,
                                  const TgsLossSpec* loss, float* partials, float* tile_loss,
-                                 int band, const uint64_t* slot_ok, const TgsRasterOpts* opts, void* stream) {
+                                 int band, const uint64_t* slot_ok, const TgsRasterOpts* opts, void* stream,
+                                 const float* ssim_adj = nullptr, float ssim_weight = 0.f, float* ssim_v_out = nullptr) {
   TGS_CHECK_ARG(camera_ok(cam), "bad camera");
   TGS_CHECK_ARG(splats && group_base && sorted_gid && tile_start && out_rgb && out_depth &&
                 final_T && partials, "null pointer");
+  if (ssim_adj) {
+    TGS_CHECK_ARG(loss && loss->gt_rgb && ssim_v_out, "the SSIM prologue needs loss->gt_rgb and the v_rgb buffer");
+    TGS_CHECK_ARG(((uintptr_t)ssim_adj & 15) == 0, "ssim_adj is not 16-byte aligned");
+    TGS_CHECK_ARG(tgs_k7_is_default_form(opts) && !slot_ok && band < 0,
+                  "the SSIM prologue exists in the default (back-to-front, one wave per tile) form of K7 only");
+  }
   LossK lk;
   lk.on = 0; lk.gt_rgb = nullptr; lk.gt_depth = nullptr; lk.unc = nullptr;
   lk.l1w = lk.dw = lk.uw = 0.f; lk.eps = 1e-6f;
@@ -2276,9 +2338,17 @@
                          v_rgb, v_depth, v_alpha, lk, partials, tile_order, qf);
       if (side) TGS_HIP(hipEventRecord(side->join, side->s));
     }
-    hipLaunchKernelGGL(k_raster_bwd, dim3(grid), dim3(64), 0, (hipStream_t)stream, k, T, splats,
-                       group_base, sorted_gid, tile_start, out_rgb, out_depth, final_T, stop_pos,
-                       v_rgb, v_depth, v_alpha, lk, partials, tile_loss, tile_order, qf);
+    if (ssim_adj) {
+      const SsimK sk{ssim_adj, loss->gt_rgb, ssim_v_out, ssim_weight, tgs_ssim_adj_pitch(cam->W), tgs_ssim_adj_plane(cam->W, cam->H)};
+      hipLaunchKernelGGL(k_raster_bwd<true>, dim3(grid), dim3(64), 0, (hipStream_t)stream, k, T, splats,
+                         group_base, sorted_gid, tile_start, out_rgb, out_depth, final_T, stop_pos,
+                         nullptr, v_depth, v_alpha, lk, partials, tile_loss, tile_order, qf, sk);
+      v_rgb = ssim_v_out;
+    } else {
+      hipLaunchKernelGGL(k_raster_bwd<false>, dim3(grid), dim3(64), 0, (hipStream_t)stream, k, T, splats,
+                         group_base, sorted_gid, tile_start, out_rgb, out_depth, final_T, stop_pos,
+                         v_rgb, v_depth, v_alpha, lk, partials, tile_loss, tile_order, qf, SsimK{});
+    }
     if (qf.factor > 0) {
       TGS_CHECK_LAUNCH();
       hipLaunchKernelGGL(k_raster_bwd_quad, dim3(min(grid, 1280)), dim3(256), 0, (hipStream_t)stream, k, T, splats,
@@ -2300,6 +2370,18 @@
                                  const TgsLossSpec* loss, float* partials, float* tile_loss,
                                  const uint64_t* slot_ok, const TgsRasterOpts* opts, void* stream) {
   return rasterize_bwd_impl(cam, splats, group_base, sorted_gid, tile_start, tile_start_len, tile_order, out_rgb, out_depth, final_T, stop_pos, v_rgb, v_depth, v_alpha, loss, partials, tile_loss, -1, slot_ok, opts, stream);
+}
+
+extern "C" int tgs_rasterize_bwd_ssim(const TgsCamera* cam, const float* splats,
+                                      const int32_t* group_base, const int32_t* sorted_gid,
+                                      int32_t* tile_start, int64_t tile_start_len, const int32_t* tile_order,
+                                      const float* out_rgb, const float* out_depth,
+                                      const float* final_T, const int32_t* stop_pos, float* v_rgb,
+                                      const float* v_depth, const float* v_alpha,
+                                      const TgsLossSpec* loss, float* partials, float* tile_loss,
+                                      const float* ssim_adj, float ssim_weight, const TgsRasterOpts* opts, void* stream) {
+  TGS_CHECK_ARG(ssim_adj, "null ssim_adj");
+  return rasterize_bwd_impl(cam, splats, group_base, sorted_gid, tile_start, tile_start_len, tile_order, out_rgb, out_depth, final_T, stop_pos, nullptr, v_depth, v_alpha, loss, partials, tile_loss, -1, nullptr, opts, stream, ssim_adj, ssim_weight, v_rgb);
 }
 
 extern "C" int tgs_rasterize_bwd_band(const TgsCamera* cam, const float* splats,
diff --git a/touch_gs_amd/csrc/tgs_ssim.h b/touch_gs_amd/csrc/tgs_ssim.h
--- /dev/null
+++ b/touch_gs_amd/csrc/tgs_ssim.h
@@ -0,0 +1,83 @@
+#pragma once
+#include <type_traits>
+#include "tgs_common.h"
+
+constexpr int TGS_SSIM_WIN = 11, TGS_SSIM_HALO = 5;
+__device__ constexpr float TGS_SSIM_WGT[TGS_SSIM_WIN] = {
+    0x1.0d956cp-10f, 0x1.f1fe02p-8f, 0x1.26eb18p-5f, 0x1.bff0fep-4f, 0x1.b43c4p-3f, 0x1.10656p-2f,
+    0x1.b43c4p-3f,   0x1.bff0fep-4f, 0x1.26eb18p-5f, 0x1.f1fe02p-8f, 0x1.0d956cp-10f};
+
+__host__ __device__ inline int tgs_ssim_adj_pitch(int W) { return (W + TGS_BLOCK - 1) / TGS_BLOCK * TGS_BLOCK + 16; }
+__host__ __device__ inline int tgs_ssim_adj_rows(int H) { return (H + TGS_BLOCK - 1) / TGS_BLOCK * TGS_BLOCK + 2 * TGS_SSIM_HALO; }
+__host__ __device__ inline size_t tgs_ssim_adj_plane(int W, int H) { return (size_t)tgs_ssim_adj_pitch(W) * tgs_ssim_adj_rows(H); }
+
+__device__ __forceinline__ float tgs_ssim_combine(float weight, float o0, float o1, float o2, float img, float gt) {
+  return weight * fmaf(o2, gt, fmaf(o1, img + img, o0));
+}
+
+constexpr int TGS_SSIM_HBUF = (TGS_BLOCK + 2 * TGS_SSIM_HALO) * TGS_BLOCK;
+
+#ifndef TGS_SSIM_DEPTH
+#define TGS_SSIM_DEPTH 2
+#endif
+template <class F>
+__device__ __forceinline__ void tgs_ssim_bwd_tile(const float* __restrict__ win, int pitch, size_t plane, int lane,
+                                                  float* __restrict__ hbuf, F&& channel_done) {
+  constexpr int ROUNDS = 18, DEPTH = TGS_SSIM_DEPTH, NROW = TGS_BLOCK + 2 * TGS_SSIM_HALO;
+  const int q4 = 4 * (lane & 3);
+  const int row[2] = {lane >> 2, min((lane >> 2) + 16, NROW - 1)};
+  const float* src[2] = {win + (size_t)row[0] * pitch + q4, win + (size_t)row[1] * pitch + q4};
+  const float* vp = hbuf + (lane >> 3) * TGS_BLOCK + (lane & 7);
+  float4 b0[DEPTH], b1[DEPTH], b2[DEPTH];
+  float2 b3[DEPTH];
+  auto issue = [&](int i, int slot) {
+    const float* s = src[i & 1] + (size_t)(i >> 1) * plane;
+    b0[slot] = ld4(s); b1[slot] = ld4(s + 4); b2[slot] = ld4(s + 8);
+    b3[slot] = *reinterpret_cast<const float2*>(s + 12);
+  };
+#pragma unroll
+  for (int i = 0; i < DEPTH; i++) issue(i, i);
+  float o[4][3];
+#pragma unroll
+  for (int i = 0; i < ROUNDS; i++) {
+    const int h = i & 1, m = (i >> 1) % 3, slot = i % DEPTH;
+    const float4 i0 = b0[slot], i1 = b1[slot], i2 = b2[slot];
+    const float2 i3 = b3[slot];
+    const float in[14] = {i0.x, i0.y, i0.z, i0.w, i1.x, i1.y, i1.z, i1.w, i2.x, i2.y, i2.z, i2.w, i3.x, i3.y};
+    float hs[4];
+#pragma unroll
+    for (int j = 0; j < 4; j++) {
+      float a = 0.f;
+#pragma unroll
+      for (int k = 0; k < TGS_SSIM_WIN; k++) a = fmaf(TGS_SSIM_WGT[k], in[j + k], a);
+      asm volatile("" : "+v"(a));
+      hs[j] = a;
+    }
+    st4(hbuf + row[h] * TGS_BLOCK + q4, make_float4(hs[0], hs[1], hs[2], hs[3]));
+    if (i + DEPTH < ROUNDS) issue(i + DEPTH, slot);
+    __builtin_amdgcn_sched_barrier(0);
+    if (h == 1) {
+      __builtin_amdgcn_fence(__ATOMIC_RELEASE, "wavefront");
+      __builtin_amdgcn_wave_barrier();
+      __builtin_amdgcn_fence(__ATOMIC_ACQUIRE, "wavefront");
+#pragma unroll
+      for (int kk = 0; kk < 4; kk++) {
+        const float* hp = vp + (8 * (kk >> 1)) * TGS_BLOCK + 8 * (kk & 1);
+        float a = 0.f;
+#pragma unroll
+        for (int k = 0; k < TGS_SSIM_WIN; k++) a = fmaf(TGS_SSIM_WGT[k], hp[k * TGS_BLOCK], a);
+        asm volatile("" : "+v"(a));
+        o[kk][m] = a;
+        __builtin_amdgcn_sched_barrier(0);
+      }
+      __builtin_amdgcn_fence(__ATOMIC_RELEASE, "wavefront");
+      __builtin_amdgcn_wave_barrier();
+      __builtin_amdgcn_fence(__ATOMIC_ACQUIRE, "wavefront");
+      if (m == 2) {
+        if (i == 5) channel_done(std::integral_constant<int, 0>{}, o);
+        else if (i == 11) channel_done(std::integral_constant<int, 1>{}, o);
+        else channel_done(std::integral_constant<int, 2>{}, o);
+      }
+    }
+  }
+}
diff --git a/touch_gs_amd/model.py b/touch_gs_amd/model.py
--- a/touch_gs_amd/model.py
+++ b/touch_gs_amd/model.py
@@ -21,6 +21,7 @@
     ssim_lambda: float = 0.2
     pipeline_ssim: bool = False
     pipeline_ssim_min_tiles: int = 0
+    fuse_ssim_bwd: bool = True
     depth_loss_mult: float = 0.2
     depth_loss_type: str = "DEPTH_UNCERTAINTY_WEIGHTED_LOSS"
     uncertainty_weight: float = 1.0
@@ -304,11 +305,18 @@
                 cam, splats, group_base, sorted_gid, tile_start, rgb, depth_acc, fT, view.rgb,
                 -c.ssim_lambda / (3 * H * W), self.loss_spec(view), self._side_stream)
         else:
-            if c.ssim_lambda > 0:
+            ssim_adj = None
+            if c.ssim_lambda > 0 and c.fuse_ssim_bwd and ops.k7_is_default_form(None, tile_start):
+                key = (W, H, rgb.device)
+                if getattr(self, "_ssim_adj", None) is None or self._ssim_adj[0] != key:
+                    self._ssim_adj = (key, ops.ssim_adj_buffer(W, H, rgb.device))
+                ssim_sum, ssim_adj = ops.ssim_fwd_adjoint(rgb, view.rgb, adj=self._ssim_adj[1])
+            elif c.ssim_lambda > 0:
                 ssim_sum, v_img = ops.ssim_fwd_bwd(rgb, view.rgb, weight=-c.ssim_lambda / (3 * H * W), reduce=False)
             partials, tile_loss = ops.rasterize_bwd(cam, splats, group_base, sorted_gid, tile_start, rgb,
                                                     depth_acc, fT, v_rgb=v_img, v_depth=v_depth, v_alpha=v_alpha,
-                                                    loss=self.loss_spec(view), want_tile_loss=True)
+                                                    loss=self.loss_spec(view), want_tile_loss=True,
+                                                    ssim_adj=ssim_adj, ssim_weight=-c.ssim_lambda / (3 * H * W))
         if fuse_adam:
             v_xy = self.optimizer.backward_and_step(cam, deg, splats, group_base, partials, want_v_xy,
                                                     begin=begin_step, guard=guard, prefetch=prefetch)
diff --git a/touch_gs_amd/ops.py b/touch_gs_amd/ops.py
--- a/touch_gs_amd/ops.py
+++ b/touch_gs_amd/ops.py
@@ -319,7 +319,8 @@
 
 def rasterize_bwd(cam: Camera, splats, group_base, sorted_gid, tile_start, rgb, depth, fT,
                   v_rgb=None, v_depth=None, v_alpha=None, loss: Optional[dict] = None,
-                  want_tile_loss: bool = False, stop_pos=None, partials=None, opts=None):
+                  want_tile_loss: bool = False, stop_pos=None, partials=None, opts=None,
+                  ssim_adj=None, ssim_weight: float = 0.0):
     lib = _lib.load()
     dev = splats.device
     _check_tile_start(tile_start, cam.num_tiles)
@@ -332,6 +333,22 @@
     if loss is not None:
         ls = _loss_spec_struct(loss, keep)
     v_rgb, v_depth, v_alpha = _f32c(v_rgb), _f32c(v_depth), _f32c(v_alpha)
+    if ssim_adj is not None:
+        H, W = cam.H, cam.W
+        if ssim_adj.dtype != torch.float32 or ssim_adj.numel() < lib.tgs_ssim_adj_len(W, H):
+            raise ValueError("ssim_adj must be the float32 buffer of ssim_fwd_adjoint for this image size")
+        if v_rgb is None:
+            v_rgb = torch.empty(H, W, 3, dtype=torch.float32, device=dev)
+        elif tuple(v_rgb.shape) != (H, W, 3):
+            raise ValueError(f"v_rgb (scratch of the SSIM prologue) must be [{H},{W},3]")
+        check(lib.tgs_rasterize_bwd_ssim(C.byref(cs), ptr(splats), ptr(group_base), ptr(sorted_gid),
+                                         ptr(tile_start), _tile_start_len(tile_start), ptr(getattr(tile_start, "tile_order", None)),
+                                         ptr(rgb), ptr(depth), ptr(fT), ptr(_stop_pos_of(fT, stop_pos)),
+                                         ptr(v_rgb), ptr(v_depth), ptr(v_alpha),
+                                         C.byref(ls) if ls is not None else None, ptr(partials), ptr(tile_loss),
+                                         ptr(ssim_adj), C.c_float(ssim_weight),
+                                         C.byref(opts) if opts is not None else None, _stream()), "tgs_rasterize_bwd_ssim")
+        return partials, tile_loss
     check(lib.tgs_rasterize_bwd(C.byref(cs), ptr(splats), ptr(group_base), ptr(sorted_gid),
                                 ptr(tile_start), _tile_start_len(tile_start), ptr(getattr(tile_start, "tile_order", None)),
                                 ptr(rgb), ptr(depth), ptr(fT), ptr(_stop_pos_of(fT, stop_pos)),
@@ -340,6 +357,12 @@
                                 ptr(tile_loss), ptr(getattr(tile_start, "slot_ok", None)),
                                 C.byref(opts) if opts is not None else None, _stream()), "tgs_rasterize_bwd")
     return partials, tile_loss
+
+
+def k7_is_default_form(opts=None, tile_start=None) -> bool:
+    if tile_start is not None and getattr(tile_start, "slot_ok", None) is not None:
+        return False
+    return bool(_lib.load().tgs_k7_is_default_form(C.byref(opts) if opts is not None else None))
 
 
 def set_raster_variant(k6_blocks: Optional[bool] = None, k7_front_to_back: Optional[bool] = None) -> int:
@@ -736,6 +759,23 @@
     return (bp.sum() if reduce else bp), v_img
 
 
+def ssim_adj_buffer(W: int, H: int, device) -> torch.Tensor:
+    return torch.zeros(_lib.load().tgs_ssim_adj_len(W, H), dtype=torch.float32, device=device)
+
+
+def ssim_fwd_adjoint(img, gt, adj=None, reduce: bool = False):
+    lib = _lib.load()
+    img, gt = _f32c(img), _f32c(gt)
+    H, W = img.shape[0], img.shape[1]
+    if adj is None:
+        adj = ssim_adj_buffer(W, H, img.device)
+    elif adj.dtype != torch.float32 or adj.numel() < lib.tgs_ssim_adj_len(W, H) or adj.device != img.device:
+        raise ValueError("adj must be a buffer of ssim_adj_buffer(W, H, device) for this image size")
+    bp = torch.empty(((H + 15) // 16) * ((W + 15) // 16), dtype=torch.float32, device=img.device)
+    check(lib.tgs_ssim_fwd_adjoint(W, H, ptr(img), ptr(gt), ptr(bp), ptr(adj), _stream()), "tgs_ssim_fwd_adjoint")
+    return (bp.sum() if reduce else bp), adj
+
+
 def depth_corr_fwd_bwd(depth_acc, final_T, mono, alpha_min: float = 0.5, weight: float = 1.0, want_grad: bool = True):
     lib = _lib.load()
     depth_acc, final_T, mono = _f32c(depth_acc.detach()), _f32c(final_T.detach()), _f32c(mono)
```

Measured after the change: 1001 iters/s (median of 6 runs). Within noise of the previous version (+0.6%).
